# openxrlab/xrsfm

Hardware: AMD Instinct MI355X
Metric: BA iterations/sec x (cams+points) (higher is better)
Workload: dtype f64

## Files before the change

include/xrsfm_ba.h:

```cpp
#ifndef XRSFM_BA_H
#define XRSFM_BA_H

#include <stddef.h>
#include <stdint.h>

#ifdef __cplusplus
extern "C" {
#endif

#define XRSFM_BA_VERSION 1

#define XRSFM_BA_OK 0
#define XRSFM_BA_EINVAL (-1)
#define XRSFM_BA_ENODEV (-2)
#define XRSFM_BA_ENOMEM (-3)
#define XRSFM_BA_ECOMM (-4)
#define XRSFM_BA_ESTATE (-5)
#define XRSFM_BA_ETOOBIG (-6)
#define XRSFM_BA_EINTERNAL (-7)
#define XRSFM_BA_ESINGULAR (-8)

#define XRSFM_BA_SIMPLE_PINHOLE 0
#define XRSFM_BA_PINHOLE 1
#define XRSFM_BA_SIMPLE_RADIAL 2
// ... 121 lines not shown
    const int32_t *sc_a, *sc_b;
    const double *sc_s12;
} xrsfm_pg_problem;

typedef struct xrsfm_pg_options {
    int32_t max_iterations;
    double function_tolerance, parameter_tolerance, gradient_tolerance;
    double initial_radius;
    int32_t verbose;
    int32_t bounds_active_set;
} xrsfm_pg_options;

typedef struct xrsfm_pg_summary {
    double initial_cost, final_cost;
    int32_t iterations, n_successful, n_unsuccessful;
    int32_t termination;
} xrsfm_pg_summary;

void xrsfm_pg_default_options(xrsfm_pg_options *opt);
int xrsfm_pg_solve(const xrsfm_pg_options *opt, xrsfm_pg_problem *problem, xrsfm_pg_summary *summary);

typedef struct xrsfm_tag_problem {
    int32_t n_frames;
    const double *frame_q;
    const double *frame_t;
    int32_t n_tags;
    double tag_length;
    double *tag_corners;
    double *tag_q, *tag_t;
    double scale;
    double scale_lower;
    int32_t n_tag_obs;
    const int32_t *tag_obs_tag, *tag_obs_frame;
    const double *tag_obs_xy;
    int32_t n_points, n_obs;
    double *points;
    const int32_t *obs_frame, *obs_pt;
    const double *obs_xy;
} xrsfm_tag_problem;

void xrsfm_tag_default_options(xrsfm_pg_options *opt);
int xrsfm_tag_refine(const xrsfm_pg_options *opt, xrsfm_tag_problem *problem, int32_t stages, xrsfm_pg_summary *summaries);

int xrsfm_ba_filter_tracks(const xrsfm_ba_problem *problem, double max_reproj_error, double min_tri_angle_rad,
                           uint8_t *obs_delete, uint8_t *track_outlier, double *track_error, double *track_angle,
                           int32_t *num_filtered);

int xrsfm_ba_profile_entry(xrsfm_ba_context *ctx, int index, const char **name, double *total_ms, int *launches);


int xrsfm_ba_debug_linearize(xrsfm_ba_context *ctx, double huber_a, int use_scaling, double *r, double *Jc,
                             double *Jp, double *Hpp, double *gp, double *Hcc_diag, double *gc, double *cost);

int xrsfm_ba_debug_schur_product(xrsfm_ba_context *ctx, double radius, const double *x, double *y, double *b);

int xrsfm_ba_debug_pack(const xrsfm_ba_problem *problem, int32_t stats[8], int32_t *slot_obs);

int xrsfm_ba_debug_sgroup(const xrsfm_ba_problem *problem, int G, int32_t stats[3], int32_t *pos_tile, int32_t *pos_code,
                          int32_t *tile_stride, int32_t *tile_cams, int32_t *tile_cidx, int32_t *cam_ptr_s);
int xrsfm_ba_debug_pack_gram(const xrsfm_ba_problem *problem, int32_t stats[8], int32_t *tile_ncam, uint8_t *slot_cidx,
                             int32_t *slot_campos_g);

int xrsfm_ba_debug_gram_schedule(int n_cams, int32_t *n_inst, int32_t *n_inst_all, uint16_t *entries);

int xrsfm_ba_debug_chol_plan(const xrsfm_ba_problem *problem, int32_t stats[8], int32_t *cam_offset, int32_t *facts);

int xrsfm_ba_debug_device_pack_check(const xrsfm_ba_problem *problem, int32_t *field, int32_t *index);

int xrsfm_ba_debug_set_block_pattern(xrsfm_ba_context *ctx, int n_pairs, const int32_t *row_col);

int xrsfm_ba_debug_cholesky_solve(xrsfm_ba_context *ctx, double radius, double *y, double *S_dense);

int xrsfm_ba_debug_reduced_system(xrsfm_ba_context *ctx, double radius, int32_t facts[16], int32_t *n_blocks, int32_t *blk_rc,
                                  double *blk, double *diag, double *b, double *y);

int xrsfm_ba_debug_wide(xrsfm_ba_context *ctx, double huber_a, double radius, double *cost, double *r, double *Jc, double *Jp,
                        double *Hcc_diag, double *gc, double *y);

int xrsfm_ba_debug_backsub(xrsfm_ba_context *ctx, double *part_model, double *part_step2, double *cand_points,
                           double *point_step, double *cand_cam_q, double *cand_cam_t);

int xrsfm_ba_debug_stored_j(xrsfm_ba_context *ctx, int32_t *stored);

#ifdef __cplusplus
}
#endif
#endif
```

xrsfm_amd/capi.py:

```python
from __future__ import annotations

import ctypes as C
import os

import numpy as np

from . import _build

_c_double_p = C.POINTER(C.c_double)
_c_int32_p = C.POINTER(C.c_int32)
_c_uint8_p = C.POINTER(C.c_uint8)


class CProblem(C.Structure):
    _fields_ = [
        ("n_cams", C.c_int32), ("n_points", C.c_int32), ("n_obs", C.c_int32), ("n_intr", C.c_int32),
        ("cam_q", _c_double_p), ("cam_t", _c_double_p), ("cam_const", _c_uint8_p), ("cam_intr", _c_int32_p),
        ("intr_model", _c_int32_p), ("intr_params", _c_double_p),
        ("points", _c_double_p), ("point_const", _c_uint8_p),
        ("obs_cam", _c_int32_p), ("obs_pt", _c_int32_p), ("obs_uv", _c_double_p),
    ]


class CPgProblem(C.Structure):
    _fields_ = [("n_frames", C.c_int32), ("n_scales", C.c_int32), ("n_edges", C.c_int32), ("n_scale_costs", C.c_int32),
                ("rot_q", _c_double_p), ("pos", _c_double_p), ("scale", _c_double_p), ("pos_const", _c_uint8_p),
                ("scale_const", _c_uint8_p), ("scale_lower", _c_double_p), ("edge_a", _c_int32_p), ("edge_b", _c_int32_p),
                ("edge_sa", _c_int32_p), ("edge_sb", _c_int32_p), ("edge_q_mea", _c_double_p), ("edge_p_mea", _c_double_p),
                ("weight_o", C.c_double), ("sc_a", _c_int32_p), ("sc_b", _c_int32_p), ("sc_s12", _c_double_p)]


class CPgOptions(C.Structure):
    _fields_ = [("max_iterations", C.c_int32), ("function_tolerance", C.c_double), ("parameter_tolerance", C.c_double),
                ("gradient_tolerance", C.c_double), ("initial_radius", C.c_double), ("verbose", C.c_int32),
                ("bounds_active_set", C.c_int32)]


class CPgSummary(C.Structure):
    _fields_ = [("initial_cost", C.c_double), ("final_cost", C.c_double), ("iterations", C.c_int32), ("n_successful", C.c_int32),
                ("n_unsuccessful", C.c_int32), ("termination", C.c_int32)]


class CTagProblem(C.Structure):
    _fields_ = [("n_frames", C.c_int32), ("frame_q", _c_double_p), ("frame_t", _c_double_p), ("n_tags", C.c_int32),
                ("tag_length", C.c_double), ("tag_corners", _c_double_p), ("tag_q", _c_double_p), ("tag_t", _c_double_p),
                ("scale", C.c_double), ("scale_lower", C.c_double), ("n_tag_obs", C.c_int32), ("tag_obs_tag", _c_int32_p),
                ("tag_obs_frame", _c_int32_p), ("tag_obs_xy", _c_double_p), ("n_points", C.c_int32), ("n_obs", C.c_int32),
                ("points", _c_double_p), ("obs_frame", _c_int32_p), ("obs_pt", _c_int32_p), ("obs_xy", _c_double_p)]


ALLREDUCE_FN = C.CFUNCTYPE(C.c_int, C.c_void_p, C.POINTER(C.c_double), C.c_uint64, C.c_int)


class COptions(C.Structure):
    _fields_ = [
        ("max_iterations", C.c_int32), ("function_tolerance", C.c_double), ("parameter_tolerance", C.c_double),
        ("gradient_tolerance", C.c_double), ("initial_radius", C.c_double), ("huber_a", C.c_double),
        ("linear_solver", C.c_int32), ("pcg_tolerance", C.c_double), ("pcg_max_iterations", C.c_int32),
        ("profile", C.c_int32), ("verbose", C.c_int32),
    ]


class CSummary(C.Structure):
    _fields_ = [
        ("initial_cost", C.c_double), ("final_cost", C.c_double),
        ("num_residuals", C.c_int32), ("num_effective_params", C.c_int32),
        ("n_successful", C.c_int32), ("n_unsuccessful", C.c_int32),
        ("termination", C.c_int32), ("termination_reason", C.c_int32),
        ("pcg_iterations", C.c_int32), ("lm_steps_attempted", C.c_int32),
        ("total_time_s", C.c_double), ("dom_kernel_ms", C.c_double),
        ("dom_kernel_launches", C.c_int32), ("dom_kernel_id", C.c_int32),
        ("linear_solver_used", C.c_int32), ("reserved", C.c_int32),
    ]

    def as_dict(self):
        return {f: getattr(self, f) for f, _ in self._fields_}


EXPORTS = [
    "xrsfm_ba_default_options", "xrsfm_ba_version", "xrsfm_ba_create", "xrsfm_ba_comm_unique_id",
    "xrsfm_ba_comm_init", "xrsfm_ba_run", "xrsfm_ba_reset", "xrsfm_ba_download", "xrsfm_ba_destroy",
    "xrsfm_ba_solve", "xrsfm_ba_filter_tracks", "xrsfm_ba_profile_entry", "xrsfm_ba_debug_linearize", "xrsfm_ba_debug_schur_product",
    "xrsfm_ba_debug_cholesky_solve", "xrsfm_ba_debug_set_block_pattern", "xrsfm_ba_debug_pack", "xrsfm_ba_debug_chol_plan", "xrsfm_ba_refine_pose", "xrsfm_ba_refine_pose_options", "xrsfm_ba_debug_comm_hook", "xrsfm_pg_default_options", "xrsfm_pg_solve", "xrsfm_ba_debug_pack_gram", "xrsfm_ba_debug_gram_schedule",
    "xrsfm_tag_default_options", "xrsfm_tag_refine", "xrsfm_ba_refine_poses", "xrsfm_ba_quiesce", "xrsfm_ba_debug_backsub", "xrsfm_ba_device_memory", "xrsfm_ba_download_intrinsics", "xrsfm_ba_debug_wide",
    "xrsfm_ba_debug_device_pack_check", "xrsfm_ba_warmup", "xrsfm_ba_debug_stored_j", "xrsfm_ba_debug_sgroup",
    "xrsfm_ba_debug_reduced_system", "xrsfm_ba_covariance",
]

CHOL_FACTS = ("T", "levels", "ordering", "schedule", "macro_levels", "split_levels", "la_depth", "fill_rest", "rest_apart", "packed",
              "bwd", "height_mask", "cw", "blocks", "n", "tiles_nz")
SCHEDULES = ("level", "panel", "lookahead")
BWD_FORMS = ("fused", "per_level", "all", "chunk", "push")


def _facts(v) -> dict:
    f = dict(zip(CHOL_FACTS, (int(x) for x in v)))
    f["schedule"] = SCHEDULES[f["schedule"]]
    f["bwd"] = BWD_FORMS[f["bwd"]]
    f["rest_apart"] = bool(f["rest_apart"]); f["packed"] = bool(f["packed"])
    f["heights"] = sorted(m * f["cw"] for m in range(1, 31) if (f["height_mask"] >> m) & 1)
    return f

SOLVER_PCG, SOLVER_CHOLESKY, SOLVER_AUTO = 0, 1, 2

ERRORS = {-1: "EINVAL", -2: "ENODEV (no HIP device / HIP error; there is no CPU fallback)", -3: "ENOMEM",
          -4: "ECOMM", -5: "ESTATE", -6: "ETOOBIG", -7: "EINTERNAL (unexpected exception inside the library)",
          -8: "ESINGULAR (the undamped reduced camera matrix is not positive definite)"}
ESINGULAR = -8

_lib = None


def load(path: str | None = None):
    global _lib
    if _lib is not None:
        return _lib
    path = path or os.environ.get("XRSFM_BA_LIB") or _build.LIB
    if not os.path.exists(path):
        raise RuntimeError(f"{path} is missing: run __graft_entry__.build() (hipcc --offload-arch=gfx950); "
                           "the BA path has no fallback implementation")
    lib = C.CDLL(path, mode=C.RTLD_GLOBAL)
    vp = C.c_void_p
    lib.xrsfm_ba_default_options.argtypes = [C.POINTER(COptions)]; lib.xrsfm_ba_default_options.restype = None
    lib.xrsfm_ba_version.argtypes = [C.POINTER(C.c_int)]; lib.xrsfm_ba_version.restype = C.c_int
    lib.xrsfm_ba_create.argtypes = [C.POINTER(CProblem), C.c_int, C.POINTER(vp)]; lib.xrsfm_ba_create.restype = C.c_int
    lib.xrsfm_ba_comm_unique_id.argtypes = [C.c_char_p]; lib.xrsfm_ba_comm_unique_id.restype = C.c_int
    lib.xrsfm_ba_comm_init.argtypes = [vp, C.c_int, C.c_int, C.c_char_p]; lib.xrsfm_ba_comm_init.restype = C.c_int
    lib.xrsfm_ba_run.argtypes = [vp, C.POINTER(COptions), C.POINTER(CSummary)]; lib.xrsfm_ba_run.restype = C.c_int
    lib.xrsfm_ba_reset.argtypes = [vp]; lib.xrsfm_ba_reset.restype = C.c_int
    lib.xrsfm_ba_download.argtypes = [vp, _c_double_p, _c_double_p, _c_double_p]; lib.xrsfm_ba_download.restype = C.c_int
    lib.xrsfm_ba_destroy.argtypes = [vp]; lib.xrsfm_ba_destroy.restype = None
    lib.xrsfm_ba_solve.argtypes = [C.POINTER(COptions), C.POINTER(CProblem), C.POINTER(CSummary)]; lib.xrsfm_ba_solve.restype = C.c_int
    lib.xrsfm_ba_filter_tracks.argtypes = [C.POINTER(CProblem), C.c_double, C.c_double, _c_uint8_p, _c_uint8_p, _c_double_p,
                                            _c_double_p, _c_int32_p]
    lib.xrsfm_ba_filter_tracks.restype = C.c_int
    lib.xrsfm_ba_debug_linearize.argtypes = [vp, C.c_double, C.c_int] + [_c_double_p] * 8
    lib.xrsfm_ba_debug_linearize.restype = C.c_int
    lib.xrsfm_ba_debug_schur_product.argtypes = [vp, C.c_double, _c_double_p, _c_double_p, _c_double_p]
    lib.xrsfm_ba_debug_schur_product.restype = C.c_int
    lib.xrsfm_ba_debug_cholesky_solve.argtypes = [vp, C.c_double, _c_double_p, _c_double_p]
    lib.xrsfm_ba_debug_cholesky_solve.restype = C.c_int
    if hasattr(lib, "xrsfm_ba_debug_stored_j"):
        lib.xrsfm_ba_debug_stored_j.argtypes = [vp, C.POINTER(C.c_int32)]
        lib.xrsfm_ba_debug_stored_j.restype = C.c_int
    if hasattr(lib, "xrsfm_ba_debug_backsub"):
        lib.xrsfm_ba_debug_backsub.argtypes = [vp] + [_c_double_p] * 6
        lib.xrsfm_ba_debug_backsub.restype = C.c_int
    lib.xrsfm_ba_debug_set_block_pattern.argtypes = [vp, C.c_int, _c_int32_p]
    lib.xrsfm_ba_debug_set_block_pattern.restype = C.c_int
    lib.xrsfm_pg_default_options.argtypes = [C.POINTER(CPgOptions)]
    lib.xrsfm_pg_default_options.restype = None
    lib.xrsfm_ba_refine_poses.argtypes = [C.POINTER(COptions), C.c_int32, _c_int32_p, _c_double_p, _c_int32_p, _c_double_p, _c_double_p,
                                          _c_uint8_p, _c_double_p, _c_double_p, C.POINTER(CSummary)]
    lib.xrsfm_ba_refine_poses.restype = C.c_int
    lib.xrsfm_pg_solve.argtypes = [C.POINTER(CPgOptions), C.POINTER(CPgProblem), C.POINTER(CPgSummary)]
    lib.xrsfm_pg_solve.restype = C.c_int
    lib.xrsfm_tag_default_options.argtypes = [C.POINTER(CPgOptions)]
    lib.xrsfm_tag_default_options.restype = None
    lib.xrsfm_tag_refine.argtypes = [C.POINTER(CPgOptions), C.POINTER(CTagProblem), C.c_int32, C.POINTER(CPgSummary)]
    lib.xrsfm_tag_refine.restype = C.c_int
    lib.xrsfm_ba_debug_comm_hook.argtypes = [C.c_void_p, C.c_int, C.c_int, ALLREDUCE_FN, C.c_void_p]
    lib.xrsfm_ba_debug_comm_hook.restype = C.c_int
    lib.xrsfm_ba_refine_pose_options.argtypes = [C.POINTER(COptions)]
    lib.xrsfm_ba_refine_pose_options.restype = None
    lib.xrsfm_ba_refine_pose.argtypes = [C.POINTER(COptions), C.c_int32, _c_double_p, C.c_int32, _c_double_p, _c_double_p, _c_uint8_p,
                                         _c_double_p, _c_double_p, C.POINTER(CSummary)]
    lib.xrsfm_ba_refine_pose.restype = C.c_int
    lib.xrsfm_ba_debug_pack_gram.argtypes = [C.POINTER(CProblem), _c_int32_p, _c_int32_p, _c_uint8_p, _c_int32_p]
    lib.xrsfm_ba_debug_pack_gram.restype = C.c_int
    lib.xrsfm_ba_debug_sgroup.argtypes = [C.POINTER(CProblem), C.c_int] + [_c_int32_p] * 7
    lib.xrsfm_ba_debug_sgroup.restype = C.c_int
    lib.xrsfm_ba_debug_chol_plan.argtypes = [C.POINTER(CProblem), _c_int32_p, _c_int32_p, _c_int32_p]
    lib.xrsfm_ba_debug_chol_plan.restype = C.c_int
    lib.xrsfm_ba_debug_reduced_system.argtypes = [vp, C.c_double, _c_int32_p, C.POINTER(C.c_int32), _c_int32_p] + [_c_double_p] * 4
    lib.xrsfm_ba_debug_reduced_system.restype = C.c_int
    lib.xrsfm_ba_debug_pack.argtypes = [C.POINTER(CProblem), _c_int32_p, _c_int32_p]
    lib.xrsfm_ba_debug_pack.restype = C.c_int
    lib.xrsfm_ba_profile_entry.argtypes = [vp, C.c_int, C.POINTER(C.c_char_p), _c_double_p, C.POINTER(C.c_int)]
    lib.xrsfm_ba_profile_entry.restype = C.c_int
    lib.xrsfm_ba_covariance.argtypes = [vp, C.c_double, C.c_int32, _c_int32_p, _c_double_p]
    lib.xrsfm_ba_covariance.restype = C.c_int
    _lib = lib
    return lib


def check(code: int, what: str):
    if code != 0:
        raise RuntimeError(f"{what} failed: {code} {ERRORS.get(code, '')}")


def _dp(a):
    return a.ctypes.data_as(_c_double_p) if a is not None else None


def device_count() -> int:
    n = C.c_int(0)
    load().xrsfm_ba_version(C.byref(n))
    return n.value


def quiesce() -> int:
    n = C.c_uint64(0)
    lib = load()
    lib.xrsfm_ba_quiesce.argtypes = [C.POINTER(C.c_uint64)]
    lib.xrsfm_ba_quiesce.restype = C.c_int
    check(lib.xrsfm_ba_quiesce(C.byref(n)), "xrsfm_ba_quiesce")
    return int(n.value)


def default_options(**kw) -> COptions:
    o = COptions()
    load().xrsfm_ba_default_options(C.byref(o))
    for k, v in kw.items():
        if not hasattr(o, k):
            raise AttributeError(k)
        setattr(o, k, v)
    return o


class ProblemArrays:
    FIELDS = ("cam_q", "cam_t", "cam_const", "cam_intr", "intr_model", "intr_params",
              "points", "point_const", "obs_cam", "obs_pt", "obs_uv")

    def __init__(self, **arr):
        f64 = lambda a, s: np.ascontiguousarray(np.asarray(a, np.float64).reshape(s))
        self.cam_q = f64(arr["cam_q"], (-1, 4)); self.cam_t = f64(arr["cam_t"], (-1, 3))
        n_c = self.cam_q.shape[0]
        cc = arr.get("cam_const")
        self.cam_const = np.ascontiguousarray(np.zeros(n_c, np.uint8) if cc is None else np.asarray(cc, np.uint8))
        self.cam_intr = np.ascontiguousarray(np.asarray(arr["cam_intr"], np.int32))
        self.intr_model = np.ascontiguousarray(np.asarray(arr["intr_model"], np.int32))
        self.intr_params = f64(arr["intr_params"], (-1, 8))
        self.points = f64(arr["points"], (-1, 3))
        pc = arr.get("point_const")
        self.point_const = np.ascontiguousarray(np.zeros(self.points.shape[0], np.uint8) if pc is None else np.asarray(pc, np.uint8))
        self.obs_cam = np.ascontiguousarray(np.asarray(arr["obs_cam"], np.int32))
        self.obs_pt = np.ascontiguousarray(np.asarray(arr["obs_pt"], np.int32))
        self.obs_uv = f64(arr["obs_uv"], (-1, 2))
        if not (self.cam_t.shape[0] == n_c and self.cam_intr.shape[0] == n_c and self.cam_const.shape[0] == n_c):
            raise ValueError("cam_q / cam_t / cam_intr / cam_const disagree on the number of cameras")
        if not (self.obs_pt.shape[0] == self.obs_cam.shape[0] == self.obs_uv.shape[0]):
            raise ValueError("obs_cam / obs_pt / obs_uv disagree on the number of observations")
        if self.point_const.shape[0] != self.points.shape[0] or self.intr_model.shape[0] != self.intr_params.shape[0]:
            raise ValueError("point_const / points or intr_model / intr_params disagree in length")

    @property
    def n_cams(self): return self.cam_q.shape[0]
    @property
    def n_points(self): return self.points.shape[0]
    @property
    def n_obs(self): return self.obs_cam.shape[0]

    def as_dict(self):
        return {k: getattr(self, k) for k in self.FIELDS}

    def c_struct(self) -> CProblem:
        i32 = lambda a: a.ctypes.data_as(_c_int32_p)
        u8 = lambda a: a.ctypes.data_as(_c_uint8_p)
        return CProblem(self.n_cams, self.n_points, self.n_obs, self.intr_model.shape[0],
                        _dp(self.cam_q), _dp(self.cam_t), u8(self.cam_const), i32(self.cam_intr),
                        i32(self.intr_model), _dp(self.intr_params), _dp(self.points), u8(self.point_const),
                        i32(self.obs_cam), i32(self.obs_pt), _dp(self.obs_uv))


class Context:

    def __init__(self, problem: ProblemArrays, device: int = 0):
        self.lib = load()
        self.problem = problem
        self._h = C.c_void_p()
        cs = problem.c_struct()
        check(self.lib.xrsfm_ba_create(C.byref(cs), device, C.byref(self._h)), "xrsfm_ba_create")

    def close(self):
        if self._h:
            self.lib.xrsfm_ba_destroy(self._h)
            self._h = C.c_void_p()

    def __del__(self):
        try:
            self.close()
        except Exception:
            pass

    def comm_init(self, n_ranks: int, rank: int, unique_id: bytes):
        check(self.lib.xrsfm_ba_comm_init(self._h, n_ranks, rank, unique_id), "xrsfm_ba_comm_init")

    def comm_hook(self, n_ranks: int, rank: int, allreduce):
        def _cb(user, buf, n, op):
            try:
                allreduce(np.ctypeslib.as_array(buf, shape=(int(n),)), int(op))
                return 0
            except Exception:
                return 1
        self._hook = ALLREDUCE_FN(_cb)
        check(self.lib.xrsfm_ba_debug_comm_hook(self._h, n_ranks, rank, self._hook, None), "xrsfm_ba_debug_comm_hook")

    def run(self, options: COptions | None = None) -> CSummary:
        options = options or default_options()
        s = CSummary()
        check(self.lib.xrsfm_ba_run(self._h, C.byref(options), C.byref(s)), "xrsfm_ba_run")
        return s

    def reset(self):
        check(self.lib.xrsfm_ba_reset(self._h), "xrsfm_ba_reset")

    def download(self, out=None):
        p = self.problem
        if out is None:
            q = np.empty_like(p.cam_q); t = np.empty_like(p.cam_t); P = p.points.copy()
        else:
            q, t, P = out
            if not (q.shape == p.cam_q.shape and t.shape == p.cam_t.shape and P.shape == p.points.shape):
                raise ValueError("download(out=...): shapes must equal the problem's cam_q / cam_t / points")
            if not all(a.dtype == np.float64 and a.flags.c_contiguous and a.flags.writeable for a in (q, t, P)):
                raise ValueError("download(out=...): arrays must be writable C-contiguous float64")
            if P is not p.points:
                P[...] = p.points
        check(self.lib.xrsfm_ba_download(self._h, _dp(q), _dp(t), _dp(P)), "xrsfm_ba_download")
        return q, t, P

    def covariance(self, cams, huber_a: float = 5.99) -> np.ndarray:
        sel = np.ascontiguousarray(cams, np.int32).reshape(-1)
        cov = np.zeros((sel.shape[0], 6, 6))
        check(self.lib.xrsfm_ba_covariance(self._h, huber_a, sel.shape[0], sel.ctypes.data_as(_c_int32_p), _dp(cov)), "xrsfm_ba_covariance")
        return cov

    def debug_linearize(self, huber_a: float = 5.99, use_scaling: bool = False):
        p = self.problem
        out = dict(r=np.zeros((p.n_obs, 2)), Jc=np.zeros((p.n_obs, 2, 6)), Jp=np.zeros((p.n_obs, 2, 3)),
                   Hpp=np.zeros((p.n_points, 6)), gp=np.zeros((p.n_points, 3)),
                   Hcc_diag=np.zeros((p.n_cams, 6)), gc=np.zeros((p.n_cams, 6)))
        cost = C.c_double(0)
        check(self.lib.xrsfm_ba_debug_linearize(self._h, huber_a, int(use_scaling), _dp(out["r"]), _dp(out["Jc"]),
                                                _dp(out["Jp"]), _dp(out["Hpp"]), _dp(out["gp"]), _dp(out["Hcc_diag"]),
                                                _dp(out["gc"]), C.cast(C.byref(cost), _c_double_p)), "debug_linearize")
        out["cost"] = cost.value
        return out

    def debug_schur_product(self, radius: float, x: np.ndarray):
        x = np.ascontiguousarray(x, np.float64)
        y = np.zeros_like(x); b = np.zeros_like(x)
        check(self.lib.xrsfm_ba_debug_schur_product(self._h, radius, _dp(x), _dp(y), _dp(b)), "debug_schur_product")
        return y, b


    def debug_stored_j(self) -> bool:
        v = C.c_int32(0)
        check(self.lib.xrsfm_ba_debug_stored_j(self._h, C.byref(v)), "debug_stored_j")
        return bool(v.value)

    def debug_cholesky_solve(self, radius: float, want_S: bool = False):
        n = 6 * self.problem.n_cams
        y = np.zeros((self.problem.n_cams, 6))
        S = np.zeros((n, n)) if want_S else None
        check(self.lib.xrsfm_ba_debug_cholesky_solve(self._h, radius, _dp(y), _dp(S)), "debug_cholesky_solve")
        return y, S

    def debug_reduced_system(self, radius: float, want_y: bool = True) -> dict:
        import scipy.sparse as sp
        lib = self.lib
        facts = np.zeros(16, np.int32)
        nb = C.c_int32(0)
        check(lib.xrsfm_ba_debug_reduced_system(self._h, radius, facts.ctypes.data_as(_c_int32_p), C.byref(nb), None, None, None, None, None),
              "xrsfm_ba_debug_reduced_system")
        f = _facts(facts)
        nc, cw, m = self.problem.n_cams, f["cw"], nb.value
        rc = np.zeros((max(m, 1), 2), np.int32); blk = np.zeros((max(m, 1), cw, cw)); diag = np.zeros((nc, cw, cw)); b = np.zeros((nc, cw))
        y = np.zeros((nc, cw)) if want_y else None
        check(lib.xrsfm_ba_debug_reduced_system(self._h, radius, facts.ctypes.data_as(_c_int32_p), C.byref(nb), rc.ctypes.data_as(_c_int32_p),
                                                _dp(blk), _dp(diag), _dp(b), _dp(y)), "xrsfm_ba_debug_reduced_system")
        rc, blk = rc[:m], blk[:m]
        ar = np.arange(cw)
        def coo(rows, cols, vals):
            shape = (len(rows), cw, cw)
            r = np.broadcast_to(cw * rows[:, None, None] + ar[None, :, None], shape)
            c = np.broadcast_to(cw * cols[:, None, None] + ar[None, None, :], shape)
            return r.ravel(), c.ravel(), vals.ravel()
        cams = np.arange(nc)
        parts = [coo(cams, cams, diag), coo(rc[:, 0], rc[:, 1], blk), coo(rc[:, 1], rc[:, 0], blk.transpose(0, 2, 1))]
        r, c, v = (np.concatenate(x) for x in zip(*parts))
        S = sp.csr_matrix((v, (r, c)), shape=(nc * cw, nc * cw))
        return dict(S=S, b=b, y=y, facts=f, blk_rc=rc)

    def download_intrinsics(self) -> np.ndarray:
        out = np.array(self.problem.intr_params, copy=True)
        self.lib.xrsfm_ba_download_intrinsics.argtypes = [C.c_void_p, _c_double_p]
        self.lib.xrsfm_ba_download_intrinsics.restype = C.c_int
        check(self.lib.xrsfm_ba_download_intrinsics(self._h, _dp(out)), "xrsfm_ba_download_intrinsics")
        return out

    def debug_wide(self, huber_a: float = 5.99, radius: float | None = None) -> dict:
        p = self.problem
        out = dict(r=np.zeros((p.n_obs, 2)), Jc=np.zeros((p.n_obs, 2, 9)), Jp=np.zeros((p.n_obs, 2, 3)), Hcc_diag=np.zeros((p.n_cams, 9)),
                   gc=np.zeros((p.n_cams, 9)))
        y = np.zeros((p.n_cams, 9)) if radius is not None else None
        cost = C.c_double(0)
        self.lib.xrsfm_ba_debug_wide.argtypes = [C.c_void_p, C.c_double, C.c_double, C.POINTER(C.c_double)] + [_c_double_p] * 6
        self.lib.xrsfm_ba_debug_wide.restype = C.c_int
        check(self.lib.xrsfm_ba_debug_wide(self._h, huber_a, float(radius or 1.0), C.byref(cost), _dp(out["r"]), _dp(out["Jc"]), _dp(out["Jp"]),
                                          _dp(out["Hcc_diag"]), _dp(out["gc"]), _dp(y)), "xrsfm_ba_debug_wide")
        out["cost"] = cost.value
        if y is not None:
            out["y"] = y
        return out

    def debug_backsub(self) -> dict:
        st = debug_pack(self.problem)
        ni, npk, nc = st["items"], st["active_points"], self.problem.n_cams
        out = dict(part_model=np.zeros(ni), part_step2=np.zeros(ni), cand_points=np.zeros((npk, 3)), point_step=np.zeros((npk, 3)),
                   cand_cam_q=np.zeros((nc, 4)), cand_cam_t=np.zeros((nc, 3)))
        check(self.lib.xrsfm_ba_debug_backsub(self._h, *[_dp(out[k]) for k in ("part_model", "part_step2", "cand_points", "point_step",
                                                                                  "cand_cam_q", "cand_cam_t")]), "debug_backsub")
        return out

    def debug_set_block_pattern(self, row_col: np.ndarray):
        rc = np.ascontiguousarray(row_col, np.int32).reshape(-1, 2)
        check(self.lib.xrsfm_ba_debug_set_block_pattern(self._h, rc.shape[0], rc.ctypes.data_as(_c_int32_p)), "debug_set_block_pattern")

    def profile(self) -> dict:
        out = {}
        i = 0
        while True:
            name = C.c_char_p(); ms = C.c_double(0); n = C.c_int(0)
            if self.lib.xrsfm_ba_profile_entry(self._h, i, C.byref(name), C.cast(C.byref(ms), _c_double_p), C.byref(n)) != 0:
                break
            out[name.value.decode()] = (ms.value, n.value)
            i += 1
        return out


def comm_unique_id() -> bytes:
    buf = C.create_string_buffer(128)
# ... 219 lines not shown
```

xrsfm_amd/csrc/ba_chol.h:

```cpp
#pragma once
#include "ba_kernels.h"
#include "ba_pack.h"

namespace xba {

constexpr int kNB = 64;
constexpr int kLdT = 66;
constexpr int kCamsPerTileDev = 10;

struct CholDev {
    int n, n_pad, T;
    double* S;
    const int* tmap; size_t ld; size_t tstride;
    double* Linv;
    double* y;
    double* rhs;
    double* x;
    const int* cam_off;
    const int* tile_rows;
    int cw, cpt;
};

__device__ __forceinline__ double* tile_ptr(const CholDev& c, int i, int k) {
    return c.tmap ? c.S + (size_t)c.tmap[i * c.T + k] * c.tstride : c.S + (size_t)(i * kNB) * c.ld + k * kNB;
// ... 204 lines not shown
    lds_ptr pb[NB];
    double acc[NB];
    lds_ptr Vb = (lds_ptr)Vst + 8 * kk;
#pragma unroll
    for (int u = 0; u < NB; ++u) {
        const int rg = e[u] & 255, cg = e[u] >> 8;
        pa[u] = Vb + 8 * (min(4 * rg + i4, R - 1) * Cp);
        pb[u] = Vb + 8 * (min(4 * cg + i4, R - 1) * Cp);
        acc[u] = 0.0;
    }
    int k0 = 0;
    for (; k0 + 16 <= C4; k0 += 16) {
#pragma unroll
        for (int j = 0; j < 4; ++j)
#pragma unroll
            for (int u = 0; u < NB; ++u)
                acc[u] = __builtin_amdgcn_mfma_f64_4x4x4f64(*(lds_dptr)(pa[u] + 32 * j), *(lds_dptr)(pb[u] + 32 * j), acc[u], 0, 0, 0);
#pragma unroll
        for (int u = 0; u < NB; ++u) { pa[u] += 128; pb[u] += 128; }
    }
    for (; k0 < C4; k0 += 4) {
#pragma unroll
        for (int u = 0; u < NB; ++u) {
            acc[u] = __builtin_amdgcn_mfma_f64_4x4x4f64(*(lds_dptr)pa[u], *(lds_dptr)pb[u], acc[u], 0, 0, 0);
            pa[u] += 32; pb[u] += 32;
        }
    }
    if (sg.len > 1 && !sgroup_finish(sg, acc, scat, lane)) return;
    int dst[NB];
    unsigned off[NB];
#pragma unroll
    for (int u = 0; u < NB; ++u) {
        const unsigned row = 4u * (unsigned)(e[u] & 255) + (unsigned)kk, col = 4u * (unsigned)(e[u] >> 8) + (unsigned)i4;
        const unsigned rb = gram_cam_of_row<CW>(row), ra = gram_cam_of_row<CW>(col);
        dst[u] = dtab[ra * kGramTabLd + rb];
        off[u] = CW * (row - CW * rb) + (col - CW * ra);
    }
#pragma unroll
    for (int u = 0; u < NB; ++u)
        if (dst[u] >= 0) scat2[(unsigned long long)(unsigned)dst[u] * (unsigned)(CW * CW) + off[u]] = acc[u];
}

template <int CW = 6>
__device__ __forceinline__ void gram_tile4(double* __restrict__ Vst, int R, int Cp, int C, const int* __restrict__ dtab,
                                           double* __restrict__ scat2, int lane, const double (&V)[3 * CW], bool valid, int t, int cidx,
                                           int T, bool dense, const unsigned short* __restrict__ sched, int n_inst, SGroup sg,
                                           double* __restrict__ scat) {
    const unsigned short* ent = sched + ((lane >> 2) & 3);
    const int C4 = (3 * T + 3) & ~3;
    if (dense) {
        const int padc = C4 - 3 * T;
        for (int e = lane; e < R * padc; e += kWave) {
            const int row = e / padc, cc = 3 * T + (e - row * padc);
            Vst[row * Cp + cc] = 0.0;
        }
    } else {
        for (int e = lane; e < (R * Cp) / 2; e += kWave) reinterpret_cast<double2*>(Vst)[e] = make_double2(0.0, 0.0);
        if (((R * Cp) & 1) && lane == kWave - 1) Vst[R * Cp - 1] = 0.0;
    }
    if (valid) {
#pragma unroll
        for (int i = 0; i < CW; ++i)
#pragma unroll
            for (int m = 0; m < 3; ++m) Vst[(CW * cidx + i) * Cp + 3 * t + m] = V[3 * i + m];
    }
    __builtin_amdgcn_s_waitcnt(0xc07f);
    __builtin_amdgcn_wave_barrier();
    XBA_STAMP(0, 6);
    switch (n_inst) {
        case 6: gram4_batch<CW, 6>(Vst, R, Cp, C4, ent, dtab, scat2, lane, sg, scat); break;
        case 5: gram4_batch<CW, 5>(Vst, R, Cp, C4, ent, dtab, scat2, lane, sg, scat); break;
        case 4: gram4_batch<CW, 4>(Vst, R, Cp, C4, ent, dtab, scat2, lane, sg, scat); break;
        case 3: gram4_batch<CW, 3>(Vst, R, Cp, C4, ent, dtab, scat2, lane, sg, scat); break;
        case 2: gram4_batch<CW, 2>(Vst, R, Cp, C4, ent, dtab, scat2, lane, sg, scat); break;
        default: gram4_batch<CW, 1>(Vst, R, Cp, C4, ent, dtab, scat2, lane, sg, scat); break;
    }
    XBA_STAMP(0, 7);
}

template <bool GRAM, bool PREP, int NIK>
__global__ __launch_bounds__((GRAM && NIK == 0) ? kWave * kSGroupMax : kWave) __attribute__((amdgpu_waves_per_eu((GRAM && NIK < 4) ? 4 : (GRAM ? 3 : 2), (GRAM && NIK < 4) ? 4 : 3)))
void k_schur_pairs(Dev d, const int* __restrict__ item_list, const int* __restrict__ slot_pair_ptr, const int* __restrict__ pair_dst,
                   int n_obs_pairs, double* __restrict__ scat2, double radius, double* __restrict__ pair_v = nullptr, int gram4 = 1,
                   const int* __restrict__ sgrp = nullptr, int n_list = 0, int wld = 0) {
    extern __shared__ __attribute__((aligned(16))) double smem_all[];
    constexpr bool MERGED = GRAM && NIK == 0;
    const int lane = MERGED ? (int)__builtin_amdgcn_mbcnt_hi(~0u, __builtin_amdgcn_mbcnt_lo(~0u, 0u)) : (int)threadIdx.x;
    const int wave = MERGED ? __builtin_amdgcn_readfirstlane((int)(threadIdx.x >> 6)) : 0;
    const int pos = MERGED ? (int)blockIdx.x * (int)(blockDim.x >> 6) + wave : (int)blockIdx.x;
    if (MERGED && pos >= n_list) return;
    double* const smem = smem_all + (size_t)wave * wld;
    XBA_STAMP(0, 0);
    SGroup sg{0, 1, smem, wld, 0.0, 0.0, -1};
    if (MERGED && sgrp) {
        const int code = __builtin_amdgcn_readfirstlane(sgrp[pos]);
        sg.idx = code & 15; sg.len = code >> 4;
    }
    const int entry = item_list[MERGED ? n_list - 1 - pos : pos];
    Item it;
    if (GRAM) { it.first_tile = entry; it.n_tiles = 1; }
    else it = d.items[entry];
    if (GRAM || it.n_tiles == 1) {
        int dt0 = -1, dt1 = -1;
        int g4_se = 0, g4_n = 0;
        if (GRAM) {
            const int C0 = d.tile_ncam[it.first_tile];
            const int* src = pair_dst + n_obs_pairs + d.tile_gt_off[it.first_tile];
            const int a0 = lane / kGramTabLd, b0 = lane - kGramTabLd * a0;
            const int a1 = (lane + kWave) / kGramTabLd, b1 = lane + kWave - kGramTabLd * a1;
            if (b0 > a0 && b0 < C0) dt0 = src[a0 * C0 + b0];
            if (b1 > a1 && b1 < C0 && a1 < kGramTabLd) dt1 = src[a1 * C0 + b1];
            if (NIK <= 2 && gram4) g4_se = gram4_sched_load<6>(C0, lane, g4_n);
        }
        const SlotCtx s = load_slot(d, it.first_tile, lane);
        const int cp = d.slot_campos_s[s.slot];
        const int cidx_raw = GRAM ? (int)d.slot_cidx[s.slot] : 0;
        const int L = d.tile_stride[it.first_tile];
        int g_pos = kWave - 1, g_pk0 = 0, g_pk1 = 0, g_pk2 = 0;
        if (GRAM && L == 0) {
            const int C0 = d.tile_ncam[it.first_tile];
            const int* trun = d.tile_run + (size_t)it.first_tile * kTileRunLd;
            const int c0 = lane / 14, c1 = (lane + 64) / 14, c2 = (lane + 128) / 14;
            g_pos = (int)d.slot_gpos[s.slot];
            if (c0 < C0) g_pk0 = trun[c0];
            if (c1 < C0) g_pk1 = trun[c1];
            if (c2 < C0) g_pk2 = trun[c2];
        }
        double V[18];
        int npair = 0, pbase = 0;
        {
            double o28[28];
            XBA_STAMP(0, 1);
            if (s.valid) {
                double hcv[6], gv[3];
                {
                    const double* hc = (PREP ? d.Hpp : d.Hc) + 6 * (size_t)s.pt;
                    const double* g = d.gp + 3 * (size_t)s.pt;
#pragma unroll
                    for (int k = 0; k < 6; ++k) hcv[k] = hc[k];
                    gv[0] = g[0]; gv[1] = g[1]; gv[2] = g[2];
                }
                double F[12], E[6], r0, r1;
                load_FE_rc(d, s.slot, s.cam, s.pt, F, E, r0, r1);
                if (PREP) { double hf[6]; point_factor(hcv, radius, hf);
#pragma unroll
                    for (int k = 0; k < 6; ++k) hcv[k] = hf[k]; }
                XBA_STAMP(0, 2);
                pairs_V<PREP>(F, E, hcv, V);
                XBA_STAMP(0, 3);
                pairs_diag<PREP>(F, V, hcv, gv, o28);
            } else if (PREP) { dead_values(V); dead_values(o28); }
            else {
#pragma unroll
                for (int k = 0; k < 18; ++k) V[k] = XBA_DEAD;
#pragma unroll
                for (int k = 0; k < 28; ++k) o28[k] = XBA_DEAD;
            }
            XBA_STAMP(0, 4);
            const int Cg = GRAM ? d.tile_ncam[it.first_tile] : 0;
            if (L > 0) {
                const int T = __popcll(__ballot(s.valid)) / L;
                double* red = smem;
#pragma unroll
                for (int h = 0; h < 2; ++h) {
#pragma unroll
                    for (int k = 0; k < 14; ++k) red[lane * kRedLd + k] = o28[14 * h + k];
                    __builtin_amdgcn_s_waitcnt(0xc07f);
                    __builtin_amdgcn_wave_barrier();
                    if ((L == 4 && T == 16) || (L == 2 && T == 32) || (L == 3 && T == 21)) {
// ... 1394 lines not shown
```

xrsfm_amd/csrc/ba_kernels.h:

```cpp
#pragma once
#include "ba_math.h"

namespace xba {

constexpr int kWave = 64;
constexpr int kBlock = 256;
constexpr int kWavesPerBlock = kBlock / kWave;

struct Item { int first_tile; int n_tiles; };

struct PcgStatus {
    double rz;
    double rr;
    double bb;
    double pq;
    int it;
    int done;
    unsigned arrived;
};

enum Scal {
    S_COST = 0, S_XNORM2_PTS, S_MODEL, S_STEP2_PTS, S_COST_CAND, S_STEP2_CAMS, S_XNORM2_CAMS,
    S_GRADMAX_PTS, S_GRADMAX_CAMS,
    S_BWD_ERR,
    S_COUNT = 16
};

struct __attribute__((aligned(16))) CamLin {
    double M[9];
    double sq[3];
    double st[3];
    double pad;
};
static_assert(sizeof(CamLin) == 128, "CamLin must be 128 bytes");

struct Dev {
    int n_cams, n_pts, n_tiles, n_slots, n_items;
    const int* slot_cam; const int* slot_pt; const int* slot_campos;
    const double* slot_u; const double* slot_v;
    const Item* items;
    const int* tile_stride;
    const int* tile_maxlen;
    const int* tile_ncam;
    const int* tile_gt_off;
    const unsigned char* slot_cidx;
    const int* slot_campos_g;
    const unsigned char* slot_gpos;
    const int* tile_run;
    const int* cam_ptr_g;
    const int* slot_campos_s; const int* cam_ptr_s;
    CamRec* cam; CamRec* cam_cand; const int* cam_model; const unsigned char* cam_const; const int* cam_ptr;
    double* cam_act;
    double* P; double* P_cand; const unsigned char* pt_const;
    double* scale_c; double* scale_p;
    double* rt; double* Jp;
    double huber_a;
    CamLin* camrec;
    double* Hpp; double* gp; double* Hinv;
    double* Hc;
    double* camlin;
    double* Dc2;
    double* camS;
    double* Minv;
    double* b;
    double* px; double* pr; double* pz; double* pp; double* pq;
    double* yp;
    double* scat;
    double* part;
    double* campart;
    double* ptpart;
    double* pcgpart;
    double* pcgW;
    double* pcgSW;
    double* pcgE;
    double* scal;
    PcgStatus* st;
};

#ifdef XBA_TIMELINE
__device__ unsigned long long g_stamps[3][64][16];
#define XBA_STAMP(kern, i) do { if ((threadIdx.x & 63) == 0 && (blockIdx.x % 97) == 0 && blockIdx.x / 97 < 64 && (threadIdx.x >> 6) == 0) g_stamps[kern][blockIdx.x / 97][i] = __builtin_readcyclecounter(); } while (0)
#define XBA_STAMP_W1(kern, i) do { if ((threadIdx.x & 63) == 0 && (blockIdx.x % 97) == 0 && blockIdx.x / 97 < 64 && (threadIdx.x >> 6) == 1) g_stamps[kern][blockIdx.x / 97][i] = __builtin_readcyclecounter(); } while (0)
#else
#define XBA_STAMP(kern, i) do {} while (0)
#define XBA_STAMP_W1(kern, i) do {} while (0)
#endif

#ifdef XBA_POISON
#define XBA_DEAD (__builtin_nan(""))
#define XBA_DEAD1 (__builtin_nan(""))
#define XBA_DEAD_VALUE(x) ((x) = __builtin_nan(""))
#else
#define XBA_DEAD 0.0
#define XBA_DEAD1 1.0
#define XBA_DEAD_VALUE(x) asm volatile("" : "=v"(x))
#endif
template <int N> __device__ __forceinline__ void dead_values(double (&v)[N]) {
#pragma unroll
    for (int k = 0; k < N; ++k) XBA_DEAD_VALUE(v[k]);
}
#ifndef XBA_BACKSUB_WAVES
#define XBA_BACKSUB_WAVES 0
#endif

__device__ __forceinline__ double wave_sum(double v) {
#pragma unroll
    for (int off = 32; off > 0; off >>= 1) v += __shfl_down(v, off, kWave);
    return v;
}
// ... 390 lines not shown
    xn2 = wave_sum(xn2);
#pragma unroll
    for (int off = 32; off > 0; off >>= 1) gm = fmax(gm, __shfl_xor(gm, off, kWave));
    if (lane == 0) { d.part[item] = cost; d.part[d.n_items + item] = xn2; d.part[2 * (size_t)d.n_items + item] = gm; }
}

__global__ __launch_bounds__(kBlock) __attribute__((amdgpu_waves_per_eu(4, 4))) void k_linearize(Dev d, double huber_a) {
    const int lane = threadIdx.x & (kWave - 1);
    const int item = __builtin_amdgcn_readfirstlane(blockIdx.x * kWavesPerBlock + (threadIdx.x >> 6));
    if (item >= d.n_items) return;
    const Item it = d.items[item];
    if (it.n_tiles > 1) linearize_item<true>(d, it, item, lane, huber_a);
    else linearize_item<false>(d, it, item, lane, huber_a);
}

__global__ __launch_bounds__(kBlock) void k_cost(Dev d, double huber_a) {
    const int lane = threadIdx.x & (kWave - 1);
    const int item = __builtin_amdgcn_readfirstlane(blockIdx.x * kWavesPerBlock + (threadIdx.x >> 6));
    if (item >= d.n_items) return;
    const Item it = d.items[item];
    double cost = 0.0;
    for (int tl = 0; tl < it.n_tiles; ++tl) {
        const int slot = (it.first_tile + tl) * kWave + lane;
        const int cam = d.slot_cam[slot];
        if (cam >= 0) {
            const CamRec& c = d.cam_cand[cam];
            double q[4] = {c.q[0], c.q[1], c.q[2], c.q[3]};
            double t[3] = {c.t[0], c.t[1], c.t[2]};
            const double* P = d.P_cand + 3 * (size_t)d.slot_pt[slot];
            const double Pw[3] = {P[0], P[1], P[2]};
            double M[9];
            quat_to_mat(q, M);
            Proj pr;
            project<false>(M, t, c.intr, d.cam_model[cam], Pw, d.slot_u[slot], d.slot_v[slot], pr);
            double rho1;
            cost += huber(pr.r0 * pr.r0 + pr.r1 * pr.r1, huber_a, rho1);
        }
    }
    cost = wave_sum(cost);
    if (lane == 0) d.part[item] = cost;
}

template <int K, bool WT = false>
__device__ __forceinline__ void segsum_body(const double* __restrict__ scat, const int* __restrict__ ptr, double* __restrict__ out, int c,
                                            double* lds_out = nullptr) {
    constexpr int G = kBlock / K;
    __shared__ double lds[G * K];
    const int t = threadIdx.x;
    const int beg = ptr[c], end = ptr[c + 1];
    if (t < G * K) {
        const int g = t / K;
        double acc = 0.0;
        const double* base = scat + (size_t)beg * K + t;
        const int n = end - beg;
        int o = g;
        for (; o + 3 * G < n; o += 4 * G) {
            const double v0 = base[0], v1 = base[(size_t)G * K], v2 = base[(size_t)2 * G * K], v3 = base[(size_t)3 * G * K];
            acc += v0; acc += v1; acc += v2; acc += v3;
            base += (size_t)4 * G * K;
        }
        for (; o < n; o += G) { acc += *base; base += (size_t)G * K; }
        lds[t] = acc;
    }
    __syncthreads();
    if (t < K) {
        double s = 0.0;
#pragma unroll 4
        for (int g = 0; g < G; ++g) s += lds[g * K + t];
        if (WT) __hip_atomic_store(out + (size_t)c * K + t, s, __ATOMIC_RELAXED, __HIP_MEMORY_SCOPE_AGENT);
        else out[(size_t)c * K + t] = s;
        if (lds_out) lds_out[t] = s;
    }
}

template <int K>
__global__ __launch_bounds__(kBlock) void k_cam_segsum(const double* __restrict__ scat, const int* __restrict__ cam_ptr,
                                                       double* __restrict__ out, const PcgStatus* st) {
    if (st && st->done) return;
    segsum_body<K>(scat, cam_ptr, out, blockIdx.x);
}

__global__ __launch_bounds__(kBlock) void k_chol_segsum(const double* __restrict__ scat, const int* __restrict__ cam_ptr,
                                                        double* __restrict__ camS, int n_cams, const double* __restrict__ scat2,
                                                        const int* __restrict__ blk_ptr, double* __restrict__ Sblk) {
    if ((int)blockIdx.x < n_cams) segsum_body<28>(scat, cam_ptr, camS, blockIdx.x);
    else segsum_body<36>(scat2, blk_ptr, Sblk, blockIdx.x - n_cams);
}

__global__ __launch_bounds__(kWave) void k_pair_sources(Dev d, const int* __restrict__ item_list, const int* __restrict__ slot_pair_ptr,
                                                        const int* __restrict__ pair_dst, int2* __restrict__ ent_src) {
    const Item it = d.items[item_list[blockIdx.x]];
    const int s_begin = it.first_tile * kWave, s_end = s_begin + it.n_tiles * kWave;
    for (int sa = s_begin + (int)threadIdx.x; sa < s_end; sa += kWave) {
        if (d.slot_cam[sa] < 0) continue;
        const int pbase = slot_pair_ptr[sa], npair = slot_pair_ptr[sa + 1] - pbase;
        for (int dd = 1; dd <= npair; ++dd) ent_src[pair_dst[pbase + dd - 1]] = make_int2(sa, sa + dd);
    }
}
__global__ __launch_bounds__(256) void k_gram_compact_count(const int* __restrict__ cell_dst, int n_cells, int* __restrict__ block_cnt) {
    const int i = blockIdx.x * 256 + threadIdx.x;
    const bool on = i < n_cells && cell_dst[i] >= 0;
    const int c = __syncthreads_count(on);
    if (threadIdx.x == 0) block_cnt[blockIdx.x] = c;
}
__global__ void k_gram_compact_scan(int* __restrict__ block_cnt, int n_blocks) {
    if (blockIdx.x != 0 || threadIdx.x != 0) return;
    int run = 0;
    for (int b = 0; b < n_blocks; ++b) { const int v = block_cnt[b]; block_cnt[b] = run; run += v; }
}
__global__ __launch_bounds__(256) void k_gram_compact(int* __restrict__ cell_dst, int n_cells, int2* __restrict__ ent_src, const int* __restrict__ block_off) {
    __shared__ int wave_cnt[4];
    const int i = blockIdx.x * 256 + threadIdx.x, lane = threadIdx.x & 63, wave = threadIdx.x >> 6;
    const int e = i < n_cells ? cell_dst[i] : -1;
    const unsigned long long m = __ballot(e >= 0);
    if (lane == 0) wave_cnt[wave] = __popcll(m);
    __syncthreads();
    if (e < 0) return;
    int rec = block_off[blockIdx.x] + __popcll(m & ((1ull << lane) - 1ull));
    for (int w = 0; w < wave; ++w) rec += wave_cnt[w];
    ent_src[e] = make_int2(-1, rec);
    cell_dst[i] = rec;
}
constexpr int kPairVAhead = 8;
__global__ __launch_bounds__(kBlock) void k_chol_segsum_v(const double* __restrict__ scat, const int* __restrict__ cam_ptr,
                                                          double* __restrict__ camS, int n_cams, const double* __restrict__ scat2,
                                                          const int* __restrict__ blk_ptr, double* __restrict__ Sblk, int n_blocks,
                                                          const int2* __restrict__ ent_src, const double* __restrict__ pair_v) {
    if ((int)blockIdx.x < n_cams) { segsum_body<28>(scat, cam_ptr, camS, blockIdx.x); return; }
    constexpr int K = 36, NW = kBlock / kWave;
    __shared__ double ops[NW][kPairVAhead][K];
    const int t = threadIdx.x, lane = t & (kWave - 1);
    const int wave = __builtin_amdgcn_readfirstlane(t >> 6);
    const int b = ((int)blockIdx.x - n_cams) * NW + wave;
    if (b >= n_blocks) return;
    const int beg = blk_ptr[b], end = blk_ptr[b + 1];
    const int k = lane < K ? lane : 0, rb3 = 3 * (k / 6), ca3 = 3 * (k % 6);
    double acc = 0.0;
    for (int e0 = beg; e0 < end; e0 += kPairVAhead) {
        const int2 mine = (lane < kPairVAhead && e0 + lane < end) ? ent_src[e0 + lane] : make_int2(-1, -1);
        int sx[kPairVAhead], sy[kPairVAhead];
        double v[kPairVAhead];
#pragma unroll
        for (int u = 0; u < kPairVAhead; ++u) {
            sx[u] = __builtin_amdgcn_readlane(mine.x, u); sy[u] = __builtin_amdgcn_readlane(mine.y, u);
            v[u] = 0.0;
            if (e0 + u < end && lane < K)
                v[u] = sx[u] < 0 ? scat2[36 * (size_t)sy[u] + lane] : pair_v[18 * (size_t)(lane < 18 ? sx[u] : sy[u]) + (lane < 18 ? lane : lane - 18)];
        }
#pragma unroll
        for (int u = 0; u < kPairVAhead; ++u) {
            if (e0 + u >= end) break;
            if (sx[u] < 0) { acc += v[u]; continue; }
            double* row = ops[wave][u];
            if (lane < K) row[lane] = v[u];
            __builtin_amdgcn_s_waitcnt(0xc07f);
            __builtin_amdgcn_wave_barrier();
            const double* Va = row + ca3;
            const double* Vb = row + 18 + rb3;
            acc += Vb[0] * Va[0] + Vb[1] * Va[1] + Vb[2] * Va[2];
        }
    }
    if (lane < K) Sblk[(size_t)b * K + lane] = acc;
}

__global__ void k_debug_materialize(Dev d, double* __restrict__ Fs, double* __restrict__ Es) {
    const int slot = blockIdx.x * blockDim.x + threadIdx.x;
    if (slot >= d.n_slots || d.slot_cam[slot] < 0) return;
    double F[12], E[6], r0, r1;
    load_FE_rc(d, slot, d.slot_cam[slot], d.slot_pt[slot], F, E, r0, r1);
    const size_t ns = (size_t)d.n_slots;
    for (int k = 0; k < 12; ++k) Fs[k * ns + slot] = F[k];
    for (int k = 0; k < 6; ++k) Es[k * ns + slot] = E[k];
}

__global__ void k_materialize_rj(Dev d, double* __restrict__ rt, double* __restrict__ Jp) {
    const int slot = blockIdx.x * blockDim.x + threadIdx.x;
    if (slot >= d.n_slots || d.slot_cam[slot] < 0) return;
    const int cam = d.slot_cam[slot];
    const CamLin& c = d.camrec[cam];
    double M[9];
    for (int k = 0; k < 9; ++k) M[k] = c.M[k];
    const double* P = d.P + 3 * (size_t)d.slot_pt[slot];
    const double Pw[3] = {P[0], P[1], P[2]};
    double r0, r1, j[6];
    obs_rj(d, slot, cam, M, Pw, r0, r1, j);
    const size_t ns = (size_t)d.n_slots;
    if (rt) { rt[slot] = r0; rt[ns + slot] = r1; }
    if (Jp) for (int k = 0; k < 6; ++k) Jp[k * ns + slot] = j[k];
}

__global__ void k_scale_from_norms(Dev d) {
    const int i = blockIdx.x * blockDim.x + threadIdx.x;
    if (i < d.n_cams * 6) {
        const int c = i / 6, k = i % 6;
        d.scale_c[i] = 1.0 / (1.0 + sqrt(d.camlin[12 * (size_t)c + k]));
    }
    if (i < d.n_pts * 3) {
        const int p = i / 3, k = i % 3;
        const int di = (k == 0) ? 0 : (k == 1 ? 3 : 5);
        d.scale_p[i] = 1.0 / (1.0 + sqrt(d.Hpp[6 * (size_t)p + di]));
    }
}

__global__ void k_fill(double* p, double v, size_t n) {
    const size_t i = (size_t)blockIdx.x * blockDim.x + threadIdx.x;
    if (i < n) p[i] = v;
}

__global__ void k_point_prep(Dev d, double radius, double dmin, double dmax, int n_pt_blocks) {
    if ((int)blockIdx.x >= n_pt_blocks) {
// ... 747 lines not shown
    if (threadIdx.x == 0) {
        double r = 0.0;
        for (int i = 0; i < kPcgThreads / kWave; ++i) r = fmax(r, lds[i]);
        *out = r;
        if (rank_max) {
            double m2 = 0.0;
            for (int i = 0; i < n_ranks; ++i) m2 = fmax(m2, rank_max[i]);
            *out_pts = m2;
        }
    }
}

struct ReduceJobs { const double* in[8]; int n[8]; double* out[8]; int op[8]; };

__global__ __launch_bounds__(kPcgThreads) void k_reduce_sum(const double* __restrict__ in, int n, double* out) {
    __shared__ double lds[kPcgThreads / kWave];
    double s = 0.0;
    for (int i = threadIdx.x; i < n; i += kPcgThreads) s += in[i];
    s = block_sum<kPcgThreads>(s, lds);
    if (threadIdx.x == 0) *out = s;
}

__global__ __launch_bounds__(kPcgThreads) void k_reduce_multi(ReduceJobs jobs) {
    __shared__ double lds[kPcgThreads / kWave];
    const double* in = jobs.in[blockIdx.x];
    const int n = jobs.n[blockIdx.x];
    if (jobs.op[blockIdx.x] == 0) {
        double s = 0.0;
        int i = threadIdx.x;
        for (; i + 7 * kPcgThreads < n; i += 8 * kPcgThreads) {
            double v[8];
#pragma unroll
            for (int u = 0; u < 8; ++u) v[u] = in[i + u * kPcgThreads];
            s += ((v[0] + v[1]) + (v[2] + v[3])) + ((v[4] + v[5]) + (v[6] + v[7]));
        }
        for (; i < n; i += kPcgThreads) s += in[i];
        s = block_sum<kPcgThreads>(s, lds);
        if (threadIdx.x == 0) *jobs.out[blockIdx.x] = s;
    } else {
        double m = 0.0;
        int i = threadIdx.x;
        for (; i + 7 * kPcgThreads < n; i += 8 * kPcgThreads) {
            double v[8];
#pragma unroll
            for (int u = 0; u < 8; ++u) v[u] = in[i + u * kPcgThreads];
#pragma unroll
            for (int u = 0; u < 8; ++u) m = fmax(m, v[u]);
        }
        for (; i < n; i += kPcgThreads) m = fmax(m, in[i]);
#pragma unroll
        for (int off = 32; off > 0; off >>= 1) m = fmax(m, __shfl_down(m, off, kWave));
        if ((threadIdx.x & 63) == 0) lds[threadIdx.x >> 6] = m;
        __syncthreads();
        if (threadIdx.x == 0) {
            double r = 0.0;
            for (int i2 = 0; i2 < kPcgThreads / kWave; ++i2) r = fmax(r, lds[i2]);
            *jobs.out[blockIdx.x] = r;
        }
    }
}

__global__ __launch_bounds__(kPcgThreads) void k_reduce_max(const double* __restrict__ in, int n, double* out) {
    __shared__ double lds[kPcgThreads / kWave];
    double m = 0.0;
    for (int i = threadIdx.x; i < n; i += kPcgThreads) m = fmax(m, in[i]);
#pragma unroll
    for (int off = 32; off > 0; off >>= 1) m = fmax(m, __shfl_down(m, off, kWave));
    if ((threadIdx.x & 63) == 0) lds[threadIdx.x >> 6] = m;
    __syncthreads();
    if (threadIdx.x == 0) {
        double r = 0.0;
        for (int i = 0; i < kPcgThreads / kWave; ++i) r = fmax(r, lds[i]);
        *out = r;
    }
}

constexpr int kTailGrid = 1024;
struct TailArgs {
    ReduceJobs jobs; int njobs;
    double* part2;
    unsigned* ticket;
    int gradmax;
    double* host; unsigned long long seq;
};

constexpr int kTailJobs = 8;

__global__ __launch_bounds__(kBlock) void k_lin_tail(Dev d, TailArgs a) {
    __shared__ double sums[12];
    __shared__ double sc[S_COUNT];
    __shared__ bool last;
    const int t = threadIdx.x, lane = t & 63, wave = t >> 6, G = gridDim.x, b = blockIdx.x;
    double gm = 0.0;
    for (int c = b; c < d.n_cams; c += G) {
        __syncthreads();
        segsum_body<12, true>(d.scat, d.cam_ptr_g, d.camlin, c, sums);
        __syncthreads();
        if (t == 0 && a.gradmax) gm = fmax(gm, cam_gradmax_one(d, c, sums + 6));
    }
    if (t == 0 && a.gradmax) __hip_atomic_store(a.part2 + (size_t)(kTailJobs - 1) * G + b, gm, __ATOMIC_RELAXED, __HIP_MEMORY_SCOPE_AGENT);
    for (int j = wave; j < a.njobs; j += kBlock / kWave) {
        const double* in = a.jobs.in[j];
        const int n = a.jobs.n[j], op = a.jobs.op[j];
        const int len = (n + G - 1) / G, lo = min(n, b * len), hi = min(n, lo + len);
        double v = 0.0;
        for (int i = lo + lane; i < hi; i += kWave) v = (op == 0) ? v + in[i] : fmax(v, in[i]);
        if (op == 0) v = wave_sum(v);
        else {
#pragma unroll
            for (int off = 32; off > 0; off >>= 1) v = fmax(v, __shfl_down(v, off, kWave));
        }
        if (lane == 0) __hip_atomic_store(a.part2 + (size_t)j * G + b, v, __ATOMIC_RELAXED, __HIP_MEMORY_SCOPE_AGENT);
    }
    asm volatile("s_waitcnt vmcnt(0)" ::: "memory");
    __syncthreads();
    if (t == 0) {
        const int sh = b & 7, nsh = min(G, 8), n_in_shard = (G - sh + 7) >> 3;
        bool l = false;
        if (__hip_atomic_fetch_add(a.ticket + 32 * sh, 1u, __ATOMIC_RELAXED, __HIP_MEMORY_SCOPE_AGENT) + 1u == (unsigned)n_in_shard)
            l = (__hip_atomic_fetch_add(a.ticket + 32 * 8, 1u, __ATOMIC_RELAXED, __HIP_MEMORY_SCOPE_AGENT) + 1u == (unsigned)nsh);
        last = l;
    }
    __syncthreads();
    if (!last) return;
    __builtin_amdgcn_fence(__ATOMIC_ACQUIRE, "agent");
    if (t < S_COUNT) sc[t] = __hip_atomic_load(d.scal + t, __ATOMIC_RELAXED, __HIP_MEMORY_SCOPE_AGENT);
    __syncthreads();
    {
        const int j = t >> 5, l32 = t & 31;
        const bool isgm = (j == kTailJobs - 1);
        const bool on = isgm ? (a.gradmax != 0) : (j < a.njobs);
        const int op = isgm ? 1 : (on ? a.jobs.op[j] : 0);
        const double* in = a.part2 + (size_t)j * G;
        double v = 0.0;
        if (on)
            for (int i0 = l32; i0 < G; i0 += 32 * 8) {
                double x[8];
#pragma unroll
                for (int u = 0; u < 8; ++u) { const int i = i0 + 32 * u; x[u] = (i < G) ? in[i] : 0.0; }
#pragma unroll
                for (int u = 0; u < 8; ++u)
                    if (i0 + 32 * u < G) v = (op == 0) ? v + x[u] : fmax(v, x[u]);
            }
#pragma unroll
        for (int off = 16; off > 0; off >>= 1) {
            const double ov = __shfl_down(v, off, 32);
            v = (op == 0) ? v + ov : fmax(v, ov);
        }
        if (on && l32 == 0) {
            double* out = isgm ? d.scal + S_GRADMAX_CAMS : a.jobs.out[j];
            *out = v;
            const long long idx = out - d.scal;
            if (idx >= 0 && idx < S_COUNT) sc[idx] = v;
        }
    }
    __syncthreads();
    if (t < 9) __hip_atomic_store(a.ticket + 32 * t, 0u, __ATOMIC_RELAXED, __HIP_MEMORY_SCOPE_AGENT);
    if (a.host) {
        if (t < S_COUNT) a.host[t] = sc[t];
        __threadfence_system();
        __syncthreads();
        if (t == 0)
            __hip_atomic_store(reinterpret_cast<unsigned long long*>(a.host + S_COUNT), a.seq, __ATOMIC_RELEASE, __HIP_MEMORY_SCOPE_SYSTEM);
    }
}

}
```

xrsfm_amd/csrc/ba_trust_region.h:

```cpp
#pragma once

#include <cmath>

#ifdef __HIPCC__
#define XTR_HD __host__ __device__
#else
#define XTR_HD
#endif

namespace xtr {

constexpr double kMaxRadius = 1e16;
constexpr double kMinRadius = 1e-32;
constexpr double kMinRelDecrease = 1e-3;
constexpr int kMaxInvalidSteps = 5;

struct TrustRegion {
    double radius;
    double decrease = 2.0;
    int invalid = 0;

    XTR_HD int invalid_step() {
        if (++invalid >= kMaxInvalidSteps) return 6;
        radius /= decrease; decrease *= 2.0;
        return 0;
    }
    XTR_HD static int tolerance_exit(double step_norm, double xnorm, double ptol, double cost_change, double cost, double ftol) {
        if (step_norm <= ptol * (xnorm + ptol)) return 2;
        if (std::fabs(cost_change) <= ftol * cost) return 3;
        return 0;
    }
    XTR_HD static bool successful(double rho) { return rho > kMinRelDecrease; }
    XTR_HD void grow(double rho) {
        radius = std::fmin(kMaxRadius, radius / std::fmax(1.0 / 3.0, 1.0 - std::pow(2.0 * rho - 1.0, 3)));
        decrease = 2.0;
    }
    XTR_HD int shrink() {
        radius /= decrease; decrease *= 2.0;
        return radius < kMinRadius ? 4 : 0;
    }
};

}
```

xrsfm_amd/csrc/xrsfm_ba.hip:

```cpp
#include <dlfcn.h>
#include <hip/hip_runtime.h>

#include <algorithm>
#include <chrono>
#include <condition_variable>
#include <deque>
#include <cmath>
#include <cstdio>
#include <cstdlib>
#include <cstring>
#include <map>
#include <mutex>
#include <thread>
#include <type_traits>
#include <vector>

#include "../../include/xrsfm_ba.h"
#include "ba_chol.h"
#include "ba_cov.h"
#include "ba_filter.h"
#include "ba_kernels.h"
#include "ba_pack.h"
#include "ba_plan.h"
#include "ba_refine.h"
// ... 66 lines not shown
    int *slot_pair_ptr = nullptr, *pair_dst = nullptr, *blk_ptr = nullptr, *blk_rc = nullptr;
    double *scat2 = nullptr, *Sblk = nullptr;
    bool bwd_push = false;
    bool bwd_chunk = false; int4* bc_chunks = nullptr; std::vector<int> bc_off; double* bc_part = nullptr; unsigned* bc_ctr = nullptr;
    int gram4 = 1;
    bool pair_from_v = false; int2* ent_src = nullptr; double* pair_v = nullptr;
    int* tiles_nz = nullptr;
    size_t pairs_shm = 0, pairs_shm_big = 0;
    int* pairs_items = nullptr; int n_pairs_small = 0, n_pairs_big = 0, n_pairs_other = 0;
    int gram_n[8] = {0}; size_t gram_shm[8] = {0};
    bool gram_merge = true;
    int sgroup = 1; int* sgrp = nullptr;
    hipStream_t aux = nullptr; hipEvent_t ev_fork = nullptr, ev_join = nullptr;
    int* cols_flat = nullptr;
    std::vector<int> cols_off;
    int* bw2_ent = nullptr; std::vector<int> bw2_off, bw2_link;
    bool use_levels = false, panel_ll = false;
    bool lookahead = false;
    int n_levels = 0;
    int *lv_k = nullptr, *lv_tgt = nullptr, *lv_cptr = nullptr, *lv_cj = nullptr;
    int *lv_bptr = nullptr, *lv_bi = nullptr;
    std::vector<int> lv_k_off, lv_tgt_off;
    int* bw_order = nullptr; unsigned char* bw_final = nullptr; unsigned long long* bw_gx = nullptr; unsigned* bw_ctr = nullptr;
    bool bw_debug_timeout = false;
    int bw_n = 0; unsigned bw_launches = 0; bool bwd_all = false;
    int *sp_tgt = nullptr, *sp_q = nullptr, *sp_rt = nullptr, *sp_rp = nullptr;
    int* sp_slot = nullptr;
    int la_depth = 0; std::vector<int> sp_e_cnt; std::vector<hipEvent_t> la_ev_factor, la_ev_early;
    std::vector<int> sp_chunk_off, sp_rt_off, mp_off;
    int *mp_chunk = nullptr, *mp_wg = nullptr;
    double* sp_work = nullptr; int sp_max_chunks = 0;
    int *fz_tile = nullptr, *fz_dptr = nullptr, *fz_dj = nullptr, *tile_cam = nullptr;
    int *md_tgt = nullptr, *md_q = nullptr, *md_cj = nullptr, *fz_late = nullptr;
    std::vector<int> md_off; int md_max = 0; double* md_work = nullptr;
    int *fz_q = nullptr, *fill_rest = nullptr; int n_fill_rest = 0;
    bool rest_apart = false;
    int32_t facts[16] = {0};
    bool S_filled = false;
    std::vector<int> fz_off;
    int *tf_ptr = nullptr, *tf_ent = nullptr;
    std::vector<int> cam_off_host;
    std::vector<int> tile_map_host; size_t S_doubles = 0;
    std::vector<int> lv_k_host, lv_bptr_host, lv_bi_host;
    int ordering = 0;
};

struct xrsfm_ba_context {
    int device = 0;
    hipStream_t stream = nullptr;
    Packed pk;
    Dev d{};
    std::vector<void*> allocs;
    std::vector<size_t> alloc_class;
    CamRec* cam0 = nullptr; double* P0 = nullptr;
    int n_points_caller = 0;
    double* h_scal = nullptr;
    double* h_scal_dev = nullptr;
    unsigned long long seq = 0;
    PcgStatus* h_st = nullptr;
    void* comm = nullptr; int n_ranks = 1, rank = 0;
    xrsfm_ba_allreduce_fn hook = nullptr; void* hook_user = nullptr; std::vector<double> hook_buf;
    bool multi() const { return comm != nullptr || hook != nullptr; }
    bool profiling = false;
    std::vector<hipEvent_t> ev_pool; size_t ev_used = 0;
    struct Rec { int kid; size_t e0; int tag; };
    std::vector<Rec> recs;
    double prof_ms[K_COUNT] = {0}; int prof_n[K_COUNT] = {0};
    bool dev_packed = false; int host_pack_level = 2;
    int* dpk_slot_obs = nullptr; unsigned char* dpk_gt_cell = nullptr;
    bool linearized = false;
    unsigned long long debug_stall_ticks = 0;
    bool poisoned = false;
    bool fused = true;
    bool wide = false;
    DevW w{};
    std::vector<int> cam_intr_host;
    bool pcg_coarse = true; double* pcg_w = nullptr;
    bool prep_fused = true;
    double step_radius = 0.0;
    bool step_prep = false;
    bool step_valid = false;
    bool gradmax_done = false, published = false;
    double* part2 = nullptr; unsigned* ticket = nullptr;
    struct LinBuf { double* rt = nullptr; double* Jp = nullptr; CamLin* camrec = nullptr; double* Hpp = nullptr; double* gp = nullptr; double* camlin = nullptr; } alt;
    double* jbuf[4] = {nullptr, nullptr, nullptr, nullptr};
    std::vector<unsigned long long> pattern_keys;
    bool have_pattern = false;
    CholHost chol;
};

namespace {

struct DevCache {
    std::mutex mu;
    std::map<std::pair<int, size_t>, std::vector<void*>> free_blocks;
    size_t cached_bytes = 0;
    static size_t size_class(size_t bytes) {
        size_t c = 256;
        while (c < bytes) c += (c < (1u << 20)) ? c : c / 4;
        return c;
    }
    void* get(int dev, size_t bytes, size_t* cls) {
        *cls = size_class(bytes);
        {
            std::lock_guard<std::mutex> g(mu);
            auto it = free_blocks.find({dev, *cls});
            if (it != free_blocks.end() && !it->second.empty()) { void* p = it->second.back(); it->second.pop_back(); cached_bytes -= *cls; return p; }
        }
        void* p = nullptr;
        if (hipMalloc(&p, *cls) != hipSuccess) {
            release_all();
            if (hipMalloc(&p, *cls) != hipSuccess) return nullptr;
        }
        return p;
    }
    void put(int dev, void* p, size_t cls) {
        std::lock_guard<std::mutex> g(mu);
        if (cached_bytes + cls > (size_t)16 << 30) { (void)hipFree(p); return; }
        free_blocks[{dev, cls}].push_back(p); cached_bytes += cls;
    }
    void release_all() {
        std::lock_guard<std::mutex> g(mu);
        for (auto& kv : free_blocks) for (void* p : kv.second) (void)hipFree(p);
        free_blocks.clear(); cached_bytes = 0;
    }
};
DevCache g_cache;

struct HostBundle { hipStream_t stream; double* h_scal; PcgStatus* h_st; hipStream_t aux = nullptr; hipEvent_t ev_fork = nullptr, ev_join = nullptr; };
static void bundle_release(const HostBundle& b) {
    (void)hipHostFree(b.h_scal); (void)hipHostFree(b.h_st); (void)hipStreamDestroy(b.stream);
    if (b.aux) { (void)hipStreamDestroy(b.aux); (void)hipEventDestroy(b.ev_fork); (void)hipEventDestroy(b.ev_join); }
}
struct BundleCache {
    std::mutex mu;
    std::map<int, std::vector<HostBundle>> free_bundles;
    bool get(int dev, HostBundle* b) {
        {
            std::lock_guard<std::mutex> g(mu);
            auto& v = free_bundles[dev];
            if (!v.empty()) { *b = v.back(); v.pop_back(); return true; }
        }
        *b = HostBundle{nullptr, nullptr, nullptr};
        if (hipStreamCreate(&b->stream) != hipSuccess) return false;
        if (hipHostMalloc((void**)&b->h_scal, sizeof(double) * (S_COUNT + 2), hipHostMallocMapped | hipHostMallocCoherent) != hipSuccess ||
            hipHostMalloc((void**)&b->h_st, sizeof(PcgStatus)) != hipSuccess) {
            if (b->h_scal) (void)hipHostFree(b->h_scal);
            (void)hipStreamDestroy(b->stream);
            return false;
        }
        return true;
    }
    void put(int dev, const HostBundle& b) {
        std::lock_guard<std::mutex> g(mu);
        auto& v = free_bundles[dev];
        if (v.size() >= 8) { bundle_release(b); return; }
        v.push_back(b);
    }
};
BundleCache g_bundles;

struct PinnedPool {
    std::mutex mu;
    std::vector<std::pair<void*, size_t>> free_blocks;
    void* get(size_t bytes, size_t* cap) {
        {
// ... 197 lines not shown
    }
    const unsigned long long* flag = reinterpret_cast<const unsigned long long*>(c->h_scal + S_COUNT);
    static const double watchdog_env = [] { const char* e = std::getenv("XRSFM_BA_WATCHDOG_S"); return e ? std::atof(e) : -1.0; }();
    const double watchdog_s = watchdog_env >= 0.0 ? watchdog_env : (c->multi() ? 300.0 : 0.0);
    std::chrono::steady_clock::time_point t_wait{};
    bool waiting = false;
    for (unsigned spins = 0; __atomic_load_n(flag, __ATOMIC_ACQUIRE) != want; ++spins) {
        if ((spins & 0xfffff) == 0xfffff) {
            const hipError_t q = hipStreamQuery(c->stream);
            if (q == hipSuccess) { if (__atomic_load_n(flag, __ATOMIC_ACQUIRE) == want) break; return XRSFM_BA_ENODEV; }
            if (q != hipErrorNotReady) return XRSFM_BA_ENODEV;
            const auto now = std::chrono::steady_clock::now();
            if (!waiting) { waiting = true; t_wait = now; }
            else if (watchdog_s > 0.0 && std::chrono::duration<double>(now - t_wait).count() > watchdog_s) {
                fprintf(stderr, "[xrsfm_ba] rank %d of %d: the device has made no progress for %.0f s%s\n", c->rank, c->n_ranks, watchdog_s,
                        c->multi() ? " — an all-reduce that never completed? every rank must make the same calls in the same order (XRSFM_BA_WATCHDOG_S)" : "");
                c->poisoned = true;
                return c->multi() ? XRSFM_BA_ECOMM : XRSFM_BA_ENODEV;
            }
        }
        __builtin_ia32_pause();
    }
    return bwd_err_check(c);
}

constexpr int kJfreeMinSlots = 1 << 20;
int jfree_setting() {
    const char* e = std::getenv("XRSFM_BA_JFREE");
    return e ? (e[0] == '0' ? 0 : 1) : -1;
}
bool jfree_enabled() { return jfree_setting() != 0; }
int use_stored_j(xrsfm_ba_context* c, bool on, bool materialize = false) {
    Dev& d = c->d;
    if (!on) { d.rt = d.Jp = c->alt.rt = c->alt.Jp = nullptr; return 0; }
    if (d.Jp) return 0;
    const size_t ns = (size_t)d.n_slots;
    for (int i = 0; i < 4; ++i) {
        if (c->jbuf[i]) continue;
        if (int e = dev_alloc(c, &c->jbuf[i], ns * (i & 1 ? 6 : 2))) { c->jbuf[i] = nullptr; return e; }
    }
    d.rt = c->jbuf[0]; d.Jp = c->jbuf[1]; c->alt.rt = c->jbuf[2]; c->alt.Jp = c->jbuf[3];
    if (materialize && ns) {
        hipLaunchKernelGGL(k_materialize_rj, dim3(cdiv((long long)ns, kBlock)), dim3(kBlock), 0, c->stream, d, d.rt, d.Jp);
        if (hipGetLastError() != hipSuccess) return XRSFM_BA_ENODEV;
    }
    return 0;
}

bool jfree_for_run(const xrsfm_ba_context* c, int solver) {
    const int set = jfree_setting();
    return solver == XRSFM_BA_SOLVER_CHOLESKY && !c->wide && c->chol.n_pairs_other == 0 && (set == 1 || (set < 0 && c->d.n_slots >= kJfreeMinSlots));
}

enum { LIN_SKIP_CAMLIN = 1, LIN_FINAL = 2 };
int linearize(xrsfm_ba_context* c, double huber_a, const Dev& d, bool with_step, int flags = 0) {
    const Dev& own = c->d;
    c->gradmax_done = false; c->published = false;
    c->step_valid = false;
    c->d.huber_a = huber_a;
    if (d.n_cams > 0 && !(flags & LIN_SKIP_CAMLIN)) LAUNCH(c, K_SMALL, k_cam_lin, dim3(cdiv(d.n_cams, kBlock)), dim3(kBlock), 0, d);
    if (d.n_items > 0) LAUNCH(c, K_LINEARIZE, k_linearize, dim3(cdiv(d.n_items, kWavesPerBlock)), dim3(kBlock), kWavesPerBlock * kWave * 13 * sizeof(double), d, huber_a);
    if (!c->fused && d.n_cams > 0) LAUNCH(c, K_CAM_SEGSUM, k_cam_segsum<12>, dim3(d.n_cams), dim3(kBlock), 0, d.scat, d.cam_ptr_g, d.camlin, (const PcgStatus*)nullptr);
    {
        double* tail = d.camlin + (size_t)d.n_cams * 12;
        const bool multi = c->multi();
        ReduceJobs j{};
        int nj = 0;
        auto job = [&](const double* in, int n, double* out, int op) { j.in[nj] = in; j.n[nj] = n; j.out[nj] = out; j.op[nj] = op; ++nj; };
        job(d.part, d.n_items, multi ? tail : d.scal + S_COST, 0);
        job(d.part + d.n_items, d.n_items, multi ? tail + 1 : d.scal + S_XNORM2_PTS, 0);
        job(d.part + 2 * (size_t)d.n_items, d.n_items, multi ? tail + 4 + c->rank : d.scal + S_GRADMAX_PTS, 1);
        if (with_step) {
            job(own.part + 2 * (size_t)own.n_items, own.n_items, multi ? tail + 2 : d.scal + S_MODEL, 0);
            job(own.part + 3 * (size_t)own.n_items, own.n_items, multi ? tail + 3 : d.scal + S_STEP2_PTS, 0);
            job(own.campart, own.n_cams, d.scal + S_STEP2_CAMS, 0);
            job(own.campart + own.n_cams, own.n_cams, d.scal + S_XNORM2_CAMS, 0);
        }
        if (multi) HIPCHK(hipMemsetAsync(tail + 2, 0, sizeof(double) * (2 + (size_t)c->n_ranks), c->stream));
        if (c->fused) {
            TailArgs a{};
            a.jobs = j; a.njobs = nj; a.part2 = c->part2; a.ticket = c->ticket;
            const bool final_here = (flags & LIN_FINAL) && !multi;
            a.gradmax = final_here ? 1 : 0;
            if (final_here && !c->profiling && c->h_scal_dev) { a.host = c->h_scal_dev; a.seq = ++c->seq; c->published = true; }
            LAUNCH(c, K_SMALL, k_lin_tail, dim3(std::min(kTailGrid, std::max(d.n_cams, 1))), dim3(kBlock), 0, d, a);
            if (final_here) c->gradmax_done = true;
        } else {
            LAUNCH(c, K_SMALL, k_reduce_multi, dim3(nj), dim3(kPcgThreads), 0, j);
        }
        if (multi) {
            int e = allreduce(c, d.camlin, (size_t)d.n_cams * 12 + 4 + (size_t)c->n_ranks, kNcclSum);
            if (e) return e;
            HIPCHK(hipMemcpyAsync(d.scal + S_COST, tail, 4 * sizeof(double), hipMemcpyDeviceToDevice, c->stream));
        }
    }
    return 0;
}

int linearize_wide(xrsfm_ba_context* c, double huber_a) {
    if (int e = use_stored_j(c, true)) return e;
    Dev& d = c->d;
    c->gradmax_done = false; c->published = false;
    if (d.n_items > 0) LAUNCH(c, K_LINEARIZE, k9_linearize, dim3(cdiv(d.n_items, kWavesPerBlock)), dim3(kBlock), 0, d, c->w, huber_a);
    if (d.n_cams > 0) LAUNCH(c, K_CAM_SEGSUM, k_cam_segsum<18>, dim3(d.n_cams), dim3(kBlock), 0, c->w.scat, d.cam_ptr_g, c->w.camlin, (const PcgStatus*)nullptr);
    ReduceJobs j{};
    const double* ins[3] = {d.part, d.part + d.n_items, d.part + 2 * (size_t)d.n_items};
    double* outs[3] = {d.scal + S_COST, d.scal + S_XNORM2_PTS, d.scal + S_GRADMAX_PTS};
    for (int q = 0; q < 3; ++q) { j.in[q] = ins[q]; j.n[q] = d.n_items; j.out[q] = outs[q]; j.op[q] = q == 2 ? 1 : 0; }
    LAUNCH(c, K_SMALL, k_reduce_multi, dim3(3), dim3(kPcgThreads), 0, j);
    return 0;
}

int gradient_max_enqueue(xrsfm_ba_context* c, const Dev& d) {
    if (c->gradmax_done) { c->gradmax_done = false; return 0; }
    if (c->wide) { LAUNCH(c, K_SMALL, k9_gradmax_cams, dim3(1), dim3(kPcgThreads), 0, d, c->w, d.scal + S_GRADMAX_CAMS); return 0; }
    const double* rank_max = c->multi() ? d.camlin + (size_t)d.n_cams * 12 + 4 : nullptr;
    LAUNCH(c, K_SMALL, k_gradmax_cams, dim3(1), dim3(kPcgThreads), 0, d, d.scal + S_GRADMAX_CAMS, rank_max, c->n_ranks, d.scal + S_GRADMAX_PTS);
    return 0;
}
int gradient_max(xrsfm_ba_context* c, double* out) {
    int e = gradient_max_enqueue(c, c->d);
    if (e) return e;
    e = fetch_scalars(c);
    if (e) return e;
    *out = std::fmax(c->h_scal[S_GRADMAX_PTS], c->h_scal[S_GRADMAX_CAMS]);
    return 0;
}

int prepare_step(xrsfm_ba_context* c, double radius, bool with_blocks = false) {
    Dev& d = c->d;
    const double dmin = kLmDiagMin, dmax = kLmDiagMax;
    c->step_radius = radius;
    c->step_prep = with_blocks && c->prep_fused;
    if (c->step_prep) return 0;
    if (!with_blocks && !d.Jp) return XRSFM_BA_EINTERNAL;
    {
        const int nbp = cdiv(d.n_pts, kBlock), nbc = cdiv((long long)d.n_cams * 6, kBlock);
        if (nbp + nbc > 0) LAUNCH(c, K_SMALL, k_point_prep, dim3(nbp + nbc), dim3(kBlock), 0, d, radius, dmin, dmax, nbp);
    }
    if (with_blocks) return 0;
    if (d.n_slots > 0) LAUNCH(c, K_SCHUR_PREP, k_schur_prep, dim3(cdiv(d.n_slots, kBlock)), dim3(kBlock), 0, d);
    if (d.n_cams > 0) LAUNCH(c, K_CAM_SEGSUM, k_cam_segsum<28>, dim3(d.n_cams), dim3(kBlock), 0, d.scat, d.cam_ptr, d.camS, (const PcgStatus*)nullptr);
    int e = allreduce(c, d.camS, (size_t)d.n_cams * 28, kNcclSum);
    if (e) return e;
    if (d.n_cams > 0) LAUNCH(c, K_SMALL, k_cam_factor, dim3(cdiv(d.n_cams, 64)), dim3(64), 0, d);
    return 0;
}

int schur_product(xrsfm_ba_context* c, const double* p_dev, double* out_dev, int tag) {
    Dev& d = c->d;
    if (d.n_items > 0) { Timed t_(c, K_SCHUR_MATVEC, tag); hipLaunchKernelGGL(k_schur_matvec, dim3(cdiv(d.n_items, kWavesPerBlock)), dim3(kBlock), 0, c->stream, d, p_dev); }
    if (d.n_cams > 0) { Timed t_(c, K_CAM_SEGSUM, tag); hipLaunchKernelGGL(k_cam_segsum<6>, dim3(d.n_cams), dim3(kBlock), 0, c->stream, d.scat, d.cam_ptr, out_dev, (const PcgStatus*)d.st); }
    return allreduce(c, out_dev, (size_t)d.n_cams * 6, kNcclSum);
}

int pcg_solve(xrsfm_ba_context* c, const xrsfm_ba_options& opt, xrsfm_ba_summary* sum) {
    Dev& d = c->d;
    d.pcgW = (c->pcg_coarse && d.n_cams > 0) ? c->pcg_w : nullptr;
    if (d.pcgW && d.n_cams > 0) {
        const size_t n6 = 6 * (size_t)d.n_cams;
        d.pcgSW = c->pcg_w + kGauge * n6; d.pcgE = c->pcg_w + 2 * kGauge * n6;
        LAUNCH(c, K_PCG_VEC, k_pcg_gauge, dim3(cdiv(d.n_cams, kBlock)), dim3(kBlock), 0, d);
        HIPCHK(hipMemsetAsync(d.st, 0, sizeof(PcgStatus), c->stream));
        for (int g = 0; g < kGauge; ++g) {
            int e = schur_product(c, d.pcgW + g * n6, d.pcgSW + g * n6, -1);
            if (e) return e;
        }
// ... 309 lines not shown
                hipLaunchKernelGGL(k_gram_compact_scan, dim3(1), dim3(64), 0, c->stream, block_off, nb);
                hipLaunchKernelGGL(k_gram_compact, dim3(nb), dim3(256), 0, c->stream, cells, n_cells, h.ent_src, (const int*)block_off);
                HIPCHK(hipGetLastError());
            }
        }
    }
    h.dev.n = P.n; h.dev.n_pad = P.n_pad; h.dev.T = P.T; h.dev.cam_off = d_cam_off; h.dev.tile_rows = d_tile_rows;
    h.dev.cw = P.cam_width; h.dev.cpt = P.cams_per_tile;
    const bool packed = chol_packed_storage(P);
    h.rest_apart = chol_rest_apart(P);
    chol_plan_facts(P, h.facts);
    h.dev.tmap = packed ? d_tmap : nullptr;
    h.dev.ld = packed ? (size_t)kNB : (size_t)P.n_pad;
    h.dev.tstride = (size_t)kNB * kNB + kNB;
    h.S_doubles = packed ? ((size_t)P.n_tiles_nz + 1) * h.dev.tstride : (size_t)P.n_pad * P.n_pad;
    if (h.S_doubles * sizeof(double) > kCholMaxBytes) return XRSFM_BA_ETOOBIG;
    h.tile_map_host = P.tile_map;
    TRYC(dev_alloc(c, &h.dev.S, h.S_doubles));
    TRYC(dev_alloc(c, &h.dev.Linv, (size_t)P.T * kNB * kNB));
    TRYC(dev_alloc(c, &h.dev.y, (size_t)P.n_pad)); TRYC(dev_alloc(c, &h.dev.rhs, (size_t)P.n_pad)); TRYC(dev_alloc(c, &h.dev.x, (size_t)P.n_pad));
    {
        const BwdChoice bw = chol_bwd_choice(P);
        h.bwd_all = bw.all; h.bwd_chunk = bw.chunk; h.bwd_push = bw.push;
        { const char* te = std::getenv("XRSFM_BA_DEBUG_BWD_TIMEOUT"); h.bw_debug_timeout = te && te[0] == '1'; }
        if (h.bwd_chunk) {
            std::vector<int4> chunks;
            h.bc_off.assign(P.n_levels + 1, 0);
            int max_lv = 1;
            for (int lv = 0; lv < P.n_levels; ++lv) {
                for (int e2 = P.lv_k_off[lv]; e2 < P.lv_k_off[lv + 1]; ++e2) {
                    const int q0 = P.lv_bptr[e2], q1 = P.lv_bptr[e2 + 1];
                    const int nch = std::max(1, (q1 - q0 + kBwdChunk - 1) / kBwdChunk);
                    for (int j = 0; j < nch; ++j) chunks.push_back(make_int4(e2, q0 + j * kBwdChunk, std::min(q1, q0 + (j + 1) * kBwdChunk), j | (nch << 16)));
                }
                h.bc_off[lv + 1] = (int)chunks.size();
                max_lv = std::max(max_lv, h.bc_off[lv + 1] - h.bc_off[lv]);
            }
            TRYC(dev_upload(c, &h.bc_chunks, chunks));
            TRYC(dev_alloc(c, &h.bc_part, (size_t)max_lv * kNB)); TRYC(dev_alloc(c, &h.bc_ctr, (size_t)P.T));
            HIPCHK(hipMemsetAsync(h.bc_ctr, 0, sizeof(unsigned) * (size_t)P.T, c->stream));
        }
        if (h.bwd_all) {
            std::vector<int> order;
            std::vector<unsigned char> fin(P.T, 0);
            for (int lv = P.n_levels - 2; lv >= 0; --lv)
                for (int e2 = P.lv_k_off[lv]; e2 < P.lv_k_off[lv + 1]; ++e2) order.push_back(e2);
            for (int e2 = P.lv_k_off[P.n_levels - 1]; e2 < P.lv_k_off[P.n_levels]; ++e2) fin[P.lv_k[e2]] = 1;
            h.bw_n = (int)order.size(); h.bw_launches = 0;
            TRYC(dev_upload(c, &h.bw_order, order)); TRYC(dev_upload(c, &h.bw_final, fin));
            TRYC(dev_alloc(c, &h.bw_gx, (size_t)P.T * 2 * kNB)); TRYC(dev_alloc(c, &h.bw_ctr, (size_t)2));
            HIPCHK(hipMemsetAsync(h.bw_gx, 0, sizeof(unsigned long long) * (size_t)P.T * 2 * kNB, c->stream));
            HIPCHK(hipMemsetAsync(h.bw_ctr, 0, sizeof(unsigned) * 2, c->stream));
        }
    }
#undef TRYC
    HIPCHK(hipMemsetAsync(h.dev.S, 0, sizeof(double) * h.S_doubles, c->stream));
    const int shm = 2 * kNB * kLdT * (int)sizeof(double);
    set_kernel_attributes(c->device);
    if ((h.n_pairs_other > 0 || h.la_depth > 0) && !h.aux) {
        if (hipStreamCreateWithFlags(&h.aux, hipStreamNonBlocking) != hipSuccess) h.aux = nullptr;
        if (h.aux && (hipEventCreateWithFlags(&h.ev_fork, hipEventDisableTiming) != hipSuccess ||
                      hipEventCreateWithFlags(&h.ev_join, hipEventDisableTiming) != hipSuccess)) {
            if (h.ev_fork) (void)hipEventDestroy(h.ev_fork);
            (void)hipStreamDestroy(h.aux); h.aux = nullptr; h.ev_fork = h.ev_join = nullptr;
        }
    }
    if (h.la_depth > 0) {
        bool ok = h.aux != nullptr;
        h.la_ev_factor.assign(h.n_levels, nullptr); h.la_ev_early.assign(h.n_levels, nullptr);
        for (int lv = 0; lv < h.n_levels && ok; ++lv)
            ok = hipEventCreateWithFlags(&h.la_ev_factor[lv], hipEventDisableTiming) == hipSuccess &&
                 hipEventCreateWithFlags(&h.la_ev_early[lv], hipEventDisableTiming) == hipSuccess;
        if (!ok) {
            for (hipEvent_t e2 : h.la_ev_factor) if (e2) (void)hipEventDestroy(e2);
            for (hipEvent_t e2 : h.la_ev_early) if (e2) (void)hipEventDestroy(e2);
            h.la_ev_factor.clear(); h.la_ev_early.clear();
        }
    }
    timer.mark("allocations + attributes");
    h.ready = true;
    return 0;
}

int chol_assemble(xrsfm_ba_context* c, bool materialize = false) {
    Dev& d = c->d;
    CholHost& h = c->chol;
    const int n_obs_pairs = h.n_pairs - c->pk.n_gt_cells;
    {
        Timed t_(c, K_SCHUR_PAIRS);
        const bool fork = h.n_pairs_other > 0 && h.aux;
        const double radius = c->step_radius;
        auto launch_other = [&](hipStream_t st) {
            const int* items = h.pairs_items + h.n_pairs_small + h.n_pairs_big;
            double* pv = h.pair_from_v ? h.pair_v : nullptr;
            if (c->step_prep) hipLaunchKernelGGL((k_schur_pairs<false, true, 0>), dim3(h.n_pairs_other), dim3(kWave), h.pairs_shm, st, d, items, h.slot_pair_ptr, h.pair_dst, n_obs_pairs, h.scat2, radius, pv);
            else hipLaunchKernelGGL((k_schur_pairs<false, false, 0>), dim3(h.n_pairs_other), dim3(kWave), h.pairs_shm, st, d, items, h.slot_pair_ptr, h.pair_dst, n_obs_pairs, h.scat2, radius, pv);
        };
        auto launch_gram = [&](auto ni, int n, size_t shm, const int* items, hipStream_t st) {
            constexpr int NI = decltype(ni)::value;
            const int G = NI == 0 ? h.sgroup : 1;
            const size_t wbytes = (shm + 15) & ~(size_t)15;
            const dim3 grid(cdiv(n, G)), block(kWave * G);
            const size_t shm_wg = G > 1 ? wbytes * G : shm;
            const int wld = G > 1 ? (int)(wbytes / sizeof(double)) : 0;
            const int* sg = G > 1 ? (const int*)h.sgrp : nullptr;
            if (c->step_prep) hipLaunchKernelGGL((k_schur_pairs<true, true, NI>), grid, block, shm_wg, st, d, items, h.slot_pair_ptr, h.pair_dst, n_obs_pairs, h.scat2, radius, (double*)nullptr, h.gram4, sg, n, wld);
            else hipLaunchKernelGGL((k_schur_pairs<true, false, NI>), grid, block, shm_wg, st, d, items, h.slot_pair_ptr, h.pair_dst, n_obs_pairs, h.scat2, radius, (double*)nullptr, h.gram4, sg, n, wld);
        };
        int n_merged = 0; size_t shm_merged = 0;
        for (int b = 0; b < 6; ++b) { n_merged += h.gram_n[b]; if (h.gram_n[b] > 0) shm_merged = std::max(shm_merged, h.gram_shm[b]); }
        const bool merge = h.gram_merge && n_merged > 0;
        constexpr bool gram_fork = true;
        int big = -1;
        for (int b = 0; b < 8; ++b) if (h.gram_n[b] > 0 && (big < 0 || h.gram_n[b] > h.gram_n[big])) big = b;
        if (merge) big = -2;
        auto launch_buckets = [&](bool main_side) {
            const int* items = h.pairs_items;
            if (merge && main_side) launch_gram(std::integral_constant<int, 0>{}, n_merged, shm_merged, items, c->stream);
            for (int b = 0; b < 8; ++b) {
                const int n = h.gram_n[b];
                const bool on_main = !(fork && gram_fork) || b == big;
                if (n > 0 && on_main == main_side && !(merge && b < 6)) {
                    hipStream_t st = on_main ? c->stream : h.aux;
                    switch (b >> 1) {
                        case 0: launch_gram(std::integral_constant<int, 1>{}, n, h.gram_shm[b], items, st); break;
                        case 1: launch_gram(std::integral_constant<int, 2>{}, n, h.gram_shm[b], items, st); break;
                        case 2: launch_gram(std::integral_constant<int, 3>{}, n, h.gram_shm[b], items, st); break;
                        default: launch_gram(std::integral_constant<int, 4>{}, n, h.gram_shm[b], items, st); break;
                    }
                }
                items += n;
            }
        };
        if (fork) {
            HIPCHK(hipEventRecord(h.ev_fork, c->stream));
            launch_buckets(true);
            HIPCHK(hipStreamWaitEvent(h.aux, h.ev_fork, 0));
            launch_other(h.aux);
            launch_buckets(false);
            HIPCHK(hipEventRecord(h.ev_join, h.aux));
            HIPCHK(hipStreamWaitEvent(c->stream, h.ev_join, 0));
        } else {
            if (h.n_pairs_other > 0) launch_other(c->stream);
            launch_buckets(true);
        }
    }
    if (d.n_cams + h.n_blocks > 0) {
        if (h.pair_from_v) LAUNCH(c, K_BLOCK_SEGSUM, k_chol_segsum_v, dim3(d.n_cams + (h.n_blocks + 3) / 4), dim3(kBlock), 0, d.scat, d.cam_ptr_s, d.camS, d.n_cams, h.scat2, h.blk_ptr, h.Sblk,
                                  h.n_blocks, (const int2*)h.ent_src, (const double*)h.pair_v);
        else LAUNCH(c, K_BLOCK_SEGSUM, k_chol_segsum, dim3(d.n_cams + h.n_blocks), dim3(kBlock), 0, d.scat, d.cam_ptr_s, d.camS, d.n_cams, h.scat2, h.blk_ptr, h.Sblk);
    }
    int e = allreduce(c, d.camS, (size_t)d.n_cams * 28 + (size_t)h.n_blocks * 36, kNcclSum);
    if (e) return e;
    h.S_filled = materialize;
    if (h.S_filled && h.n_tiles_nz > 0)
        LAUNCH(c, K_DENSE_FILL, k_tile_fill, dim3(h.n_tiles_nz), dim3(256), 0, h.dev, d, h.tiles_nz, h.tf_ptr, h.tf_ent, h.Sblk, h.blk_rc,
               c->step_prep ? c->step_radius : 0.0);
    return 0;
}

static void panel_backward(xrsfm_ba_context* c) {
    CholHost& h = c->chol;
    const int T = h.T;
    int k = T - 1;
    for (int p = 0; k >= 1; k -= 2, ++p) {
            const int n = h.bw2_off[p + 1] - h.bw2_off[p];
            LAUNCH(c, K_TRISOLVE, k_bwd2, dim3(1 + n), dim3(256), 0, h.dev, k, h.bw2_link[p], (const int*)(h.bw2_ent + 2 * (size_t)h.bw2_off[p]));
        }
    for (; k >= 0; --k) {
        const int ncol = h.cols_off[k + 1] - h.cols_off[k];
        LAUNCH(c, K_TRISOLVE, k_bwd, dim3(1 + ncol), dim3(256), 0, h.dev, k, h.cols_flat + h.cols_off[k]);
    }
}

int chol_factor_solve(xrsfm_ba_context* c) {
    Dev& d = c->d;
    CholHost& h = c->chol;
    const int T = h.T;
    double* px_out = c->wide ? c->w.px : d.px;
    const size_t shm = 2 * (size_t)kNB * kLdT * sizeof(double);
    if (h.lookahead) {
        auto chunks = [&](int lv) { return lv < h.n_levels ? h.sp_chunk_off[lv + 1] - h.sp_chunk_off[lv] : 0; };
        auto targets = [&](int lv) { return lv < h.n_levels ? h.sp_rt_off[lv + 1] - h.sp_rt_off[lv] : 0; };
        auto lates = [&](int lv) { return lv < h.n_levels ? h.md_off[lv + 1] - h.md_off[lv] : 0; };
        double* const Wbuf[2] = {h.sp_work, h.sp_work + (size_t)std::max(1, h.sp_max_chunks) * kPartStride};
        double* const Qbuf[2] = {h.md_work, h.md_work + (size_t)std::max(1, h.md_max) * kPartStride};
        for (int s2 = 0; s2 < h.n_levels; ++s2) {
            const int nf = h.fz_off[s2 + 1] - h.fz_off[s2];
            SlotArgs a{};
            const int lr = s2 + 1, lp = s2 + 2;
            a.n_reduce = targets(lr);
            if (a.n_reduce > 0) { a.sp_rt = h.sp_rt + 2 * (size_t)h.sp_rt_off[lr]; a.sp_rp = h.sp_rp + 2 * (size_t)h.sp_rt_off[lr]; a.Wr = Wbuf[lr & 1]; }
            a.n_part = chunks(lp);
            if (a.n_part > 0) { a.sp_tgt = h.sp_tgt + 2 * (size_t)h.sp_chunk_off[lp]; a.sp_q = h.sp_q + 2 * (size_t)h.sp_chunk_off[lp]; a.Wp = Wbuf[lp & 1]; }
            a.n_late = lates(lr);
            if (a.n_late > 0) { a.md_tgt = h.md_tgt + 2 * (size_t)h.md_off[lr]; a.md_q = h.md_q + 2 * (size_t)h.md_off[lr]; a.Wq = Qbuf[lr & 1]; }
            if (s2 == 0 && !h.S_filled) {
                LvFill lf{};
                lf.d = d; lf.f = FillLists{h.tiles_nz, h.tf_ptr, h.tf_ent, h.Sblk, h.blk_rc, c->step_prep ? c->step_radius : 0.0};
                lf.fz_q = h.fz_q; lf.rest = h.fill_rest; lf.n_factor = nf;
                if (nf + h.n_fill_rest > 0)
                    LAUNCH(c, K_POTRF, k_lv_factor<true>, dim3(nf + h.n_fill_rest), dim3(256), 0, h.dev, h.fz_tile, h.fz_dptr, h.fz_dj,
                           (const int*)h.tile_cam, (double*)nullptr, lf);
                if (a.n_reduce + a.n_part + a.n_late > 0) return XRSFM_BA_EINTERNAL;
                continue;
            }
            a.fz_tile = h.fz_tile + 2 * (size_t)h.fz_off[s2]; a.fz_dptr = h.fz_dptr + h.fz_off[s2]; a.n_factor = nf;
            a.fz_late = h.fz_late + 2 * (size_t)h.fz_off[s2]; a.Ql = Qbuf[s2 & 1];
            const int nwg = a.n_factor + a.n_reduce + a.n_late + a.n_part;
            if (nwg > 0) LAUNCH(c, K_POTRF, k_panel_slot, dim3(nwg), dim3(256), 0, h.dev, a, (const int*)h.fz_dj, (const int*)h.lv_cj, (const int*)h.md_cj, (const int*)h.tile_cam);
        }
        panel_backward(c);
        if (d.n_cams > 0) LAUNCH(c, K_SMALL, k_sol_gather, dim3(cdiv((long long)d.n_cams * h.dev.cw, 256)), dim3(256), 0, h.dev, px_out, d.n_cams);
        return 0;
    }
    if (h.use_levels || h.panel_ll) {
        for (int lv = 0; lv < h.n_levels; ++lv) {
            const int nt = h.lv_tgt_off[lv + 1] - h.lv_tgt_off[lv];
            const int nch = h.sp_chunk_off[lv + 1] - h.sp_chunk_off[lv], nmc = h.mp_off[lv + 1] - h.mp_off[lv] - 1;
            const int nrt = h.sp_rt_off[lv + 1] - h.sp_rt_off[lv];
            const bool la_on = h.la_depth > 0 && !h.la_ev_factor.empty();
            const int n_early = la_on ? h.sp_e_cnt[lv] : 0;
            double* const Wlv = h.sp_work + (h.la_depth > 0 ? (size_t)(lv % (h.la_depth + 1)) * (size_t)std::max(1, h.sp_max_chunks) * kPartStride : 0);
            if (nmc > 0)
                LAUNCH(c, K_UPDATE, k_panel2_part, dim3(nmc), dim3(256), 0, h.dev, h.mp_chunk, h.mp_wg + h.mp_off[lv], h.sp_work);
            else if (nch - n_early > 0)
                LAUNCH(c, K_UPDATE, k_ll_update_part, dim3(nch - n_early), dim3(256), 0, h.dev, h.sp_tgt + 2 * (size_t)(h.sp_chunk_off[lv] + n_early),
                       h.sp_q + 2 * (size_t)(h.sp_chunk_off[lv] + n_early), h.lv_cj, Wlv, (const int*)(h.sp_slot + h.sp_chunk_off[lv] + n_early));
            if (n_early > 0) HIPCHK(hipStreamWaitEvent(c->stream, h.la_ev_early[lv], 0));
            if (nrt > 0)
                LAUNCH(c, K_UPDATE, k_ll_update_reduce, dim3(nrt, 16), dim3(256), 0, h.dev, h.sp_rt + 2 * (size_t)h.sp_rt_off[lv],
                       h.sp_rp + 2 * (size_t)h.sp_rt_off[lv], Wlv);
            const int nf = h.fz_off[lv + 1] - h.fz_off[lv];
            const bool with_bwd = ((!h.panel_ll && !h.bwd_push && !h.bwd_chunk) || T == 1) && lv == h.n_levels - 1;
            LvFill lf{};
            if (lv == 0 && !h.S_filled) {
                lf.d = d; lf.f = FillLists{h.tiles_nz, h.tf_ptr, h.tf_ent, h.Sblk, h.blk_rc, c->step_prep ? c->step_radius : 0.0};
                lf.fz_q = h.fz_q; lf.rest = h.fill_rest; lf.n_factor = nf;
                const bool rest_apart = h.rest_apart;
                if (rest_apart)
                    LAUNCH(c, K_DENSE_FILL, k_tile_fill, dim3(h.n_fill_rest), dim3(256), 0, h.dev, d, h.tiles_nz, h.tf_ptr, h.tf_ent, h.Sblk, h.blk_rc,
                           c->step_prep ? c->step_radius : 0.0, (const int*)h.fill_rest);
                const int n_rest = rest_apart ? 0 : h.n_fill_rest;
                if (nf + n_rest > 0)
                    LAUNCH(c, K_POTRF, k_lv_factor<true>, dim3(nf + n_rest), dim3(256), 0, h.dev, h.fz_tile, h.fz_dptr, h.fz_dj,
                           (const int*)h.tile_cam, with_bwd ? px_out : (double*)nullptr, lf);
            } else if (nf > 0)
                LAUNCH(c, K_POTRF, k_lv_factor<false>, dim3(nf), dim3(256), 0, h.dev, h.fz_tile + 2 * (size_t)h.fz_off[lv], h.fz_dptr + h.fz_off[lv], h.fz_dj,
                       (const int*)h.tile_cam, with_bwd ? px_out : (double*)nullptr, lf);
            if (la_on) {
                const int le = lv + 1 + h.la_depth;
                const int ne = le < h.n_levels ? h.sp_e_cnt[le] : 0;
                if (ne > 0) {
                    HIPCHK(hipEventRecord(h.la_ev_factor[lv], c->stream));
                    HIPCHK(hipStreamWaitEvent(h.aux, h.la_ev_factor[lv], 0));
                    double* const Wle = h.sp_work + (size_t)(le % (h.la_depth + 1)) * (size_t)std::max(1, h.sp_max_chunks) * kPartStride;
                    {
                        Timed t_(c, K_UPDATE, -1, h.aux);
                        hipLaunchKernelGGL(k_ll_update_part, dim3(ne), dim3(256), 0, h.aux, h.dev, h.sp_tgt + 2 * (size_t)h.sp_chunk_off[le],
                                           h.sp_q + 2 * (size_t)h.sp_chunk_off[le], h.lv_cj, Wle, (const int*)(h.sp_slot + h.sp_chunk_off[le]));
                    }
                    HIPCHK(hipEventRecord(h.la_ev_early[le], h.aux));
                }
            }
        }
        if (h.panel_ll || h.bwd_push) {
            if (T == 1) return 0;
            panel_backward(c);
            if (d.n_cams > 0) LAUNCH(c, K_SMALL, k_sol_gather, dim3(cdiv((long long)d.n_cams * h.dev.cw, 256)), dim3(256), 0, h.dev, px_out, d.n_cams);
            return 0;
        }
        if (h.bwd_chunk) {
            for (int lv = h.n_levels - 1; lv >= 0; --lv) {
                const int n = h.bc_off[lv + 1] - h.bc_off[lv];
                if (n > 0) LAUNCH(c, K_TRISOLVE, k_lv_bwd_chunk, dim3(n), dim3(256), 0, h.dev, (const int*)h.lv_k, (const int*)h.lv_bi, (const int*)h.tile_cam, px_out,
                                  (const int4*)(h.bc_chunks + h.bc_off[lv]), h.bc_part, h.bc_ctr);
            }
            return 0;
        }
        if (h.bwd_all && h.bw_n > 0) {
            const unsigned base = h.bw_launches * (unsigned)h.bw_n;
            const unsigned epoch = ++h.bw_launches;
            LAUNCH(c, K_TRISOLVE, k_lv_bwd_all, dim3(h.bw_n), dim3(256), 0, h.dev, (const int*)h.lv_k, (const int*)h.lv_bptr, (const int*)h.lv_bi,
                   (const int*)h.tile_cam, px_out, (const int*)h.bw_order, (const unsigned char*)h.bw_final, h.bw_gx, h.bw_ctr, base, epoch, h.bw_ctr + 1,
                   d.scal + S_BWD_ERR, h.bw_debug_timeout ? 64u : kBwdSpinMax, h.bw_debug_timeout ? epoch + 1u : epoch);
            return 0;
        }
        for (int lv = h.n_levels - 2; lv >= 0; --lv) {
            const int nk = h.lv_k_off[lv + 1] - h.lv_k_off[lv];
            LAUNCH(c, K_TRISOLVE, k_lv_bwd, dim3(nk), dim3(256), 0, h.dev, h.lv_k + h.lv_k_off[lv], h.lv_bptr + h.lv_k_off[lv], h.lv_bi, h.tile_cam, px_out);
        }
        return 0;
    }
    return XRSFM_BA_EINTERNAL;
}

Dev candidate_view(const xrsfm_ba_context* c) {
    Dev v = c->d;
    std::swap(v.cam, v.cam_cand); std::swap(v.P, v.P_cand);
    v.rt = c->alt.rt; v.Jp = c->alt.Jp; v.camrec = c->alt.camrec; v.Hpp = c->alt.Hpp; v.gp = c->alt.gp; v.camlin = c->alt.camlin;
    v.part = c->d.part + 4 * (size_t)c->d.n_items;
    return v;
}
void accept_candidate(xrsfm_ba_context* c) {
    Dev& d = c->d;
    std::swap(d.cam, d.cam_cand); std::swap(d.P, d.P_cand);
    std::swap(d.rt, c->alt.rt); std::swap(d.Jp, c->alt.Jp); std::swap(d.camrec, c->alt.camrec);
    std::swap(d.Hpp, c->alt.Hpp); std::swap(d.gp, c->alt.gp); std::swap(d.camlin, c->alt.camlin);
}

int finish_step(xrsfm_ba_context* c, double huber_a, bool speculate) {
    Dev& d = c->d;
    const bool cams_done = c->fused;
    if (c->wide) {
        const int nbi = cdiv(d.n_items, kWavesPerBlock), nbc = cdiv(d.n_cams, kBlock);
        if (nbi + nbc > 0) LAUNCH(c, K_BACKSUB, k9_backsub, dim3(nbi + nbc), dim3(kBlock), 0, d, c->w, nbi, c->step_radius);
    } else {
        const int nbi = cdiv(d.n_items, kWavesPerBlock), nbc = cams_done ? cdiv(d.n_cams, kBlock) : 0;
        CamLin* cr = (cams_done && speculate) ? c->alt.camrec : (CamLin*)nullptr;
        if (nbi + nbc > 0) {
            if (c->step_prep) LAUNCH(c, K_BACKSUB, k_backsub<true>, dim3(nbi + nbc), dim3(kBlock), 0, d, nbi, cr, c->step_radius);
            else LAUNCH(c, K_BACKSUB, k_backsub<false>, dim3(nbi + nbc), dim3(kBlock), 0, d, nbi, cr, c->step_radius);
        }
        if (d.n_cams > 0 && !cams_done) LAUNCH(c, K_SMALL, k_cam_update, dim3(cdiv(d.n_cams, kBlock)), dim3(kBlock), 0, d);
    }
    if (speculate) {
        const Dev cand = candidate_view(c);
        int e = linearize(c, huber_a, cand, true, LIN_FINAL | (cams_done ? LIN_SKIP_CAMLIN : 0));
        if (e) return e;
        if ((e = gradient_max_enqueue(c, cand))) return e;
        return fetch_scalars(c);
    }
    if (d.n_items > 0) LAUNCH(c, K_COST, k_cost, dim3(cdiv(d.n_items, kWavesPerBlock)), dim3(kBlock), 0, d, huber_a);
    {
        ReduceJobs j{};
        const double* ins[5] = {d.part, d.part + 2 * (size_t)d.n_items, d.part + 3 * (size_t)d.n_items, d.campart, d.campart + d.n_cams};
        const int ns[5] = {d.n_items, d.n_items, d.n_items, d.n_cams, d.n_cams};
        double* outs[5] = {d.scal + S_COST_CAND, d.scal + S_MODEL, d.scal + S_STEP2_PTS, d.scal + S_STEP2_CAMS, d.scal + S_XNORM2_CAMS};
        for (int q = 0; q < 5; ++q) { j.in[q] = ins[q]; j.n[q] = ns[q]; j.out[q] = outs[q]; j.op[q] = 0; }
        LAUNCH(c, K_SMALL, k_reduce_multi, dim3(5), dim3(kPcgThreads), 0, j);
    }
    int e = allreduce(c, d.scal + S_MODEL, 3, kNcclSum);
    if (e) return e;
    return fetch_scalars(c);
}

int bwd_all_status(xrsfm_ba_context* c) {
    CholHost& h = c->chol;
    if (!h.bwd_all || h.bw_launches == 0 || !h.bw_ctr) return 0;
    unsigned ev = 0;
    if (hipMemcpy(&ev, h.bw_ctr + 1, sizeof(unsigned), hipMemcpyDeviceToHost) != hipSuccess) return XRSFM_BA_ENODEV;
    if (ev) {
        fprintf(stderr, "[xrsfm_ba] backward substitution: a hand-off between workgroups timed out (k_lv_bwd_all); rerun with XRSFM_BA_BWD_ALL=0\n");
        (void)hipMemset(h.bw_ctr + 1, 0, sizeof(unsigned));
        return XRSFM_BA_EINTERNAL;
    }
    return 0;
}

void print_progress(const xrsfm_ba_options& o, int it, double cost, double change, double gmax, double step, double rho, double radius) {
    if (!o.verbose) return;
    if (it == 0) printf("iter      cost      cost_change  |gradient|   |step|    tr_ratio  tr_radius\n");
    printf("%4d  %.6e  %9.2e  %9.2e  %9.2e  %9.2e  %9.2e\n", it, cost, change, gmax, step, rho, radius);
}

int init_scaling_and_linearize(xrsfm_ba_context* c, double huber_a, bool use_scaling) {
    Dev& d = c->d;
    const int cw = c->wide ? kW : 6;
    int e;
    LAUNCH(c, K_SMALL, k_fill, dim3(cdiv((long long)d.n_cams * cw, kBlock) + 1), dim3(kBlock), 0, c->wide ? c->w.scale_c : d.scale_c, 1.0, (size_t)d.n_cams * cw);
    LAUNCH(c, K_SMALL, k_fill, dim3(cdiv((long long)d.n_pts * 3, kBlock) + 1), dim3(kBlock), 0, d.scale_p, 1.0, (size_t)d.n_pts * 3);
    c->gradmax_done = false; c->published = false;
    auto lin = [&](int flags) { return c->wide ? linearize_wide(c, huber_a) : linearize(c, huber_a, d, false, flags); };
    if ((e = lin(use_scaling ? 0 : LIN_FINAL))) return e;
    if (use_scaling) {
        const long long n = std::max((long long)d.n_cams * cw, (long long)d.n_pts * 3);
        if (c->wide) LAUNCH(c, K_SMALL, k9_scale_from_norms, dim3(cdiv(n, kBlock) + 1), dim3(kBlock), 0, d, c->w);
        else LAUNCH(c, K_SMALL, k_scale_from_norms, dim3(cdiv(n, kBlock) + 1), dim3(kBlock), 0, d);
        if ((e = lin(LIN_FINAL))) return e;
    }
    c->linearized = true;
    return 0;
}

struct DevScratch {
    std::vector<void*> p;
    ~DevScratch() { for (void* q : p) (void)hipFree(q); }
    template <typename T>
    int get(T** out, size_t n) {
        void* q = nullptr;
        if (hipMalloc(&q, std::max<size_t>(1, n) * sizeof(T)) != hipSuccess) return XRSFM_BA_ENOMEM;
        p.push_back(q); *out = static_cast<T*>(q);
        return 0;
    }
    template <typename T>
    int put(T** out, const std::vector<T>& v) {
        if (int e = get(out, v.size())) return e;
        if (!v.empty() && hipMemcpy(*out, v.data(), v.size() * sizeof(T), hipMemcpyHostToDevice) != hipSuccess) return XRSFM_BA_ENODEV;
        return 0;
    }
};

static int cov_solution_status(xrsfm_ba_context* c, std::vector<double>& x) {
    x.resize((size_t)c->d.n_cams * 6);
    HIPCHK(hipMemcpyAsync(x.data(), c->d.px, x.size() * sizeof(double), hipMemcpyDeviceToHost, c->stream));
    HIPCHK(hipStreamSynchronize(c->stream));
    if (int e = bwd_all_status(c)) return e;
    for (double v : x) if (!std::isfinite(v)) return XRSFM_BA_ESINGULAR;
    return 0;
}

struct CovLists {
    std::vector<int4> ent; std::vector<int2> lj; std::vector<int> sel_row, sel_cam;
// ... 572 lines not shown
    }
    if (d.n_cams + h.n_blocks > 0) LAUNCH(c, K_BLOCK_SEGSUM, k9_chol_segsum, dim3(d.n_cams + h.n_blocks), dim3(kBlock), 0, c->w.scat, d.cam_ptr_g, c->w.camS, d.n_cams, h.scat2, h.blk_ptr, h.Sblk);
    if (h.n_tiles_nz > 0) LAUNCH(c, K_DENSE_FILL, k9_tile_fill, dim3(h.n_tiles_nz), dim3(256), 0, h.dev, d, c->w, h.tiles_nz, h.tf_ptr, h.tf_ent, h.Sblk, h.blk_rc, radius);
    h.S_filled = true;
    return 0;
}

static int ba_run_impl(xrsfm_ba_context* c, const xrsfm_ba_options* optp, xrsfm_ba_summary* sum) {
    if (!c || !optp || !sum) return XRSFM_BA_EINVAL;
    if (c->poisoned) return XRSFM_BA_ESTATE;
    const xrsfm_ba_options opt = *optp;
    HIPCHK(hipSetDevice(c->device));
    if (const char* se = std::getenv("XRSFM_BA_DEBUG_STALL_S"))
        c->debug_stall_ticks = (unsigned long long)(std::fmin(std::fmax(std::atof(se), 0.0), 10.0) * 1e8);
    memset(sum, 0, sizeof(*sum));
    Dev& d = c->d;
    hipStream_t st = c->stream;
    int solver = opt.linear_solver;
    int e;
    if (c->wide) {
        if (solver == XRSFM_BA_SOLVER_PCG || c->multi()) {
            fprintf(stderr, "[xrsfm_ba] variable intrinsics (9-wide camera blocks): only the exact solver on one rank is implemented\n");
            return XRSFM_BA_EINVAL;
        }
        solver = XRSFM_BA_SOLVER_CHOLESKY;
    }
    if (solver == XRSFM_BA_SOLVER_AUTO) {
        try { e = chol_setup(c); } catch (const std::bad_alloc&) { e = XRSFM_BA_ENOMEM; }
        if (e == XRSFM_BA_ETOOBIG || e == XRSFM_BA_ENOMEM || e == kErrDuplicateObs) solver = XRSFM_BA_SOLVER_PCG;
        else if (e) return e;
        else solver = XRSFM_BA_SOLVER_CHOLESKY;
    }
    if (solver != XRSFM_BA_SOLVER_PCG && solver != XRSFM_BA_SOLVER_CHOLESKY) return XRSFM_BA_EINVAL;
    if (solver == XRSFM_BA_SOLVER_CHOLESKY && (e = chol_setup(c))) {
        if (e == kErrDuplicateObs) {
            fprintf(stderr, "[xrsfm_ba] a track is observed twice by one camera: the explicit reduced camera matrix is not available, use AUTO or PCG\n");
            return XRSFM_BA_EINVAL;
        }
        return e;
    }
    if ((e = use_stored_j(c, !jfree_for_run(c, solver)))) return e;
    sum->linear_solver_used = solver;
    c->profiling = opt.profile != 0;
    for (int i = 0; i < K_COUNT; ++i) { c->prof_ms[i] = 0.0; c->prof_n[i] = 0; }
    c->recs.clear(); c->ev_used = 0;
    const auto t_begin = std::chrono::steady_clock::now();
    sum->num_residuals = 2 * c->pk.n_obs;
    {
        int n_var_i = 0;
        if (c->wide && d.n_cams) {
            std::vector<unsigned char> cc(d.n_cams);
            std::vector<double> act(d.n_cams);
            HIPCHK(hipMemcpy(cc.data(), d.cam_const, d.n_cams, hipMemcpyDeviceToHost)); HIPCHK(hipMemcpy(act.data(), d.cam_act, sizeof(double) * d.n_cams, hipMemcpyDeviceToHost));
            for (int i = 0; i < d.n_cams; ++i) n_var_i += (act[i] > 0.0 && (cc[i] & kCamIntrVariable)) ? 1 : 0;
        }
        sum->num_effective_params = 3 * (c->pk.n_var_q + c->pk.n_var_t + c->pk.n_var_p + n_var_i);
    }
    auto finish = [&](int term, int reason, double cost) {
        sum->termination = term; sum->termination_reason = reason; sum->final_cost = cost;
        (void)hipStreamSynchronize(st);
        sum->total_time_s = std::chrono::duration<double>(std::chrono::steady_clock::now() - t_begin).count();
        if (int be = bwd_all_status(c)) return be;
        if (c->profiling) {
            profile_collect(c);
            int best = 0;
            for (int i = 1; i < K_COUNT - 1; ++i) if (c->prof_ms[i] > c->prof_ms[best]) best = i;
            sum->dom_kernel_id = best; sum->dom_kernel_ms = c->prof_ms[best]; sum->dom_kernel_launches = c->prof_n[best];
        }
        c->profiling = false;
        return XRSFM_BA_OK;
    };
    if ((e = init_scaling_and_linearize(c, opt.huber_a, true))) return e;
    double gmax = 0.0;
    if ((e = gradient_max(c, &gmax))) return e;
    double cost = 0.5 * c->h_scal[S_COST];
    double xnorm2_pts = c->h_scal[S_XNORM2_PTS];
    sum->initial_cost = cost;
    xtr::TrustRegion tr{opt.initial_radius};
    print_progress(opt, 0, cost, 0.0, gmax, 0.0, 0.0, tr.radius);
    if (gmax <= opt.gradient_tolerance) return finish(XRSFM_BA_CONVERGENCE, 1, cost);
    int it = 0;
    bool speculate = !c->wide;
    int accepted_run = 0;
    while (true) {
        if (it >= opt.max_iterations) return finish(XRSFM_BA_NO_CONVERGENCE, 5, cost);
        ++it;
        sum->lm_steps_attempted++;
        if (c->wide) {
            if ((e = assemble_wide(c, tr.radius))) return e;
            if ((e = chol_factor_solve(c))) return e;
        } else {
            if ((e = prepare_step(c, tr.radius, solver == XRSFM_BA_SOLVER_CHOLESKY))) return e;
            if (solver == XRSFM_BA_SOLVER_PCG) {
                if ((e = pcg_solve(c, opt, sum))) return e;
            } else {
                if ((e = chol_assemble(c))) return e;
                if ((e = chol_factor_solve(c))) return e;
            }
        }
        if ((e = finish_step(c, opt.huber_a, speculate))) return e;
        const double* s = c->h_scal;
        const double model_change = s[S_MODEL];
        const double xnorm = std::sqrt(xnorm2_pts + s[S_XNORM2_CAMS]);
        if (!(model_change > 0.0) || !std::isfinite(model_change)) {
            sum->n_unsuccessful++;
            print_progress(opt, it, cost, 0.0, gmax, 0.0, 0.0, tr.radius);
            if (const int r = tr.invalid_step()) return finish(XRSFM_BA_FAILURE, r, cost);
            if (!d.Jp && (e = use_stored_j(c, true, true))) return e;
            continue;
        }
        tr.invalid = 0;
        const double cost_cand = 0.5 * (speculate ? s[S_COST] : s[S_COST_CAND]);
        const double step_norm = std::sqrt(s[S_STEP2_PTS] + s[S_STEP2_CAMS]);
        const double cost_change = cost - cost_cand;
        if (const int r = xtr::TrustRegion::tolerance_exit(step_norm, xnorm, opt.parameter_tolerance, cost_change, cost, opt.function_tolerance))
            return finish(XRSFM_BA_CONVERGENCE, r, cost);
        const double rel = cost_change / model_change;
        if (xtr::TrustRegion::successful(rel)) {
            if (speculate) {
                accept_candidate(c);
                cost = cost_cand;
                xnorm2_pts = s[S_XNORM2_PTS];
                gmax = std::fmax(s[S_GRADMAX_PTS], s[S_GRADMAX_CAMS]);
            } else {
                std::swap(d.cam, d.cam_cand);
                std::swap(d.P, d.P_cand);
                if ((e = c->wide ? linearize_wide(c, opt.huber_a) : linearize(c, opt.huber_a, d, false, LIN_FINAL))) return e;
                if ((e = gradient_max(c, &gmax))) return e;
                cost = 0.5 * c->h_scal[S_COST];
                xnorm2_pts = c->h_scal[S_XNORM2_PTS];
            }
            ++accepted_run;
            speculate = !c->wide && (sum->n_unsuccessful == 0 || accepted_run >= 2);
            tr.grow(rel);
            sum->n_successful++;
            print_progress(opt, it, cost, cost_change, gmax, step_norm, rel, tr.radius);
            if (gmax <= opt.gradient_tolerance) return finish(XRSFM_BA_CONVERGENCE, 1, cost);
        } else {
            speculate = false; accepted_run = 0;
            const int r = tr.shrink();
            if (!d.Jp && (e = use_stored_j(c, true, true))) return e;
            sum->n_unsuccessful++;
            print_progress(opt, it, cost, cost_change, gmax, step_norm, rel, tr.radius);
            if (r) return finish(XRSFM_BA_CONVERGENCE, r, cost);
        }
    }
}

int xrsfm_ba_profile_entry(xrsfm_ba_context* c, int index, const char** name, double* total_ms, int* launches) {
    if (!c || index < 0 || index >= K_COUNT) return XRSFM_BA_EINVAL;
    if (name) *name = kKidName[index];
    if (total_ms) *total_ms = c->prof_ms[index];
    if (launches) *launches = c->prof_n[index];
    return 0;
}

int xrsfm_ba_solve(const xrsfm_ba_options* opt, xrsfm_ba_problem* problem, xrsfm_ba_summary* summary) {
    if (!opt || !problem || !summary) return XRSFM_BA_EINVAL;
    static const bool trace = std::getenv("XRSFM_BA_TRACE_CALLS") != nullptr;
    using clk = std::chrono::steady_clock;
    const auto t0 = clk::now();
    xrsfm_ba_context* c = nullptr;
    int e = xrsfm_ba_create(problem, 0, &c);
    if (e) return e;
    const auto t1 = clk::now();
    e = xrsfm_ba_run(c, opt, summary);
    const auto t2 = clk::now();
    if (!e) e = xrsfm_ba_download(c, problem->cam_q, problem->cam_t, problem->points);
    if (!e && problem->intr_params) e = xrsfm_ba_download_intrinsics(c, problem->intr_params);
    const auto t3 = clk::now();
    xrsfm_ba_destroy(c);
    if (trace) {
        auto ms = [](clk::time_point a, clk::time_point b) { return std::chrono::duration<double, std::milli>(b - a).count(); };
        std::fprintf(stderr, "[xrsfm_ba_solve] cams %d points %d obs %d | create %.3f run %.3f download %.3f destroy %.3f ms | LM %d+%d solver %d rc %d\n",
                     problem->n_cams, problem->n_points, problem->n_obs, ms(t0, t1), ms(t1, t2), ms(t2, t3), ms(t3, clk::now()),
                     summary->n_successful, summary->n_unsuccessful, summary->linear_solver_used, e);
    }
    return e;
}

void xrsfm_pg_default_options(xrsfm_pg_options* o) {
    if (!o) return;
    o->max_iterations = 100; o->function_tolerance = 1e-6; o->parameter_tolerance = 1e-8; o->gradient_tolerance = 1e-10;
    o->initial_radius = 1e16; o->verbose = 0; o->bounds_active_set = 0;
}

static int pg_solve_impl(const xrsfm_pg_options* opt, xrsfm_pg_problem* p, xrsfm_pg_summary* summary) {
    if (!p || !summary) return XRSFM_BA_EINVAL;
    if (p->n_frames < 0 || p->n_scales < p->n_frames || p->n_edges < 0 || p->n_scale_costs < 0) return XRSFM_BA_EINVAL;
    if (p->n_frames > 0 && (!p->rot_q || !p->pos)) return XRSFM_BA_EINVAL;
    if (p->n_scales > 0 && !p->scale) return XRSFM_BA_EINVAL;
    if (p->n_edges > 0 && (!p->edge_a || !p->edge_b || !p->edge_sa || !p->edge_sb || !p->edge_q_mea || !p->edge_p_mea)) return XRSFM_BA_EINVAL;
    if (p->n_scale_costs > 0 && (!p->sc_a || !p->sc_b || !p->sc_s12)) return XRSFM_BA_EINVAL;
    for (int e = 0; e < p->n_edges; ++e) {
        if (p->edge_a[e] < 0 || p->edge_a[e] >= p->n_frames || p->edge_b[e] < 0 || p->edge_b[e] >= p->n_frames) return XRSFM_BA_EINVAL;
        if (p->edge_sa[e] < 0 || p->edge_sa[e] >= p->n_scales || p->edge_sb[e] < 0 || p->edge_sb[e] >= p->n_scales) return XRSFM_BA_EINVAL;
    }
    for (int e = 0; e < p->n_scale_costs; ++e)
        if (p->sc_a[e] < 0 || p->sc_a[e] >= p->n_scales || p->sc_b[e] < 0 || p->sc_b[e] >= p->n_scales) return XRSFM_BA_EINVAL;
    xrsfm_pg_options o;
    if (opt) o = *opt; else xrsfm_pg_default_options(&o);
    xpg::Solver solver(*p);
    return solver.run(o, summary);
}

void xrsfm_tag_default_options(xrsfm_pg_options* o) {
    if (!o) return;
    o->max_iterations = 500;
    o->function_tolerance = 1e-6; o->parameter_tolerance = 1e-8; o->gradient_tolerance = 1e-10;
    o->initial_radius = 1e4; o->verbose = 0; o->bounds_active_set = 0;
}

static int tag_refine_impl(const xrsfm_pg_options* opt, xrsfm_tag_problem* p, int32_t stages, xrsfm_pg_summary* summaries) {
    if (!p || !summaries || stages < 1 || stages > 2) return XRSFM_BA_EINVAL;
    if (p->n_frames < 0 || p->n_tags < 0 || p->n_tag_obs < 0 || p->n_points < 0 || p->n_obs < 0) return XRSFM_BA_EINVAL;
    if (p->n_frames > 0 && (!p->frame_q || !p->frame_t)) return XRSFM_BA_EINVAL;
    if (p->n_tags > 0 && (!p->tag_corners || !p->tag_q || !p->tag_t)) return XRSFM_BA_EINVAL;
    if (p->n_tag_obs > 0 && (!p->tag_obs_tag || !p->tag_obs_frame || !p->tag_obs_xy)) return XRSFM_BA_EINVAL;
    if (p->n_points > 0 && !p->points) return XRSFM_BA_EINVAL;
    if (p->n_obs > 0 && (!p->obs_frame || !p->obs_pt || !p->obs_xy)) return XRSFM_BA_EINVAL;
    if (!(p->tag_length > 0.0) || !std::isfinite(p->scale)) return XRSFM_BA_EINVAL;
    for (int i = 0; i < p->n_tag_obs; ++i)
        if (p->tag_obs_tag[i] < 0 || p->tag_obs_tag[i] >= p->n_tags || p->tag_obs_frame[i] < 0 || p->tag_obs_frame[i] >= p->n_frames) return XRSFM_BA_EINVAL;
    for (int i = 0; i < p->n_obs; ++i)
        if (p->obs_pt[i] < 0 || p->obs_pt[i] >= p->n_points || p->obs_frame[i] < 0 || p->obs_frame[i] >= p->n_frames) return XRSFM_BA_EINVAL;
    xrsfm_pg_options o;
    if (opt) o = *opt; else xrsfm_tag_default_options(&o);
    return xtag::refine(o, *p, stages, summaries);
}
// ... 755 lines not shown
```

Measured before the change: 1.127 billion.

## Decide LM step acceptance on device and queue next Schur assembly ahead

Moves the Levenberg-Marquardt accept/reject and trust-region update into the final linearization tail kernel. It writes a go word keyed by the sequence number so the next iteration's Schur-pair and segment-sum kernels can be enqueued speculatively before the host reads the scalars. Those kernels exit early when the device decides not to continue, and the radius is read from device memory. This hides the host round trip between iterations, at the cost of bit-exact replication of the host trust-region arithmetic on device, with a fallback to the host when rounding could differ.

New measurement: 1.124 billion. Within noise of the previous version (-0.3%).

```diff
diff --git a/include/xrsfm_ba.h b/include/xrsfm_ba.h
--- a/include/xrsfm_ba.h
+++ b/include/xrsfm_ba.h
@@ -227,6 +227,9 @@
 
 int xrsfm_ba_debug_stored_j(xrsfm_ba_context *ctx, int32_t *stored);
 
+int xrsfm_ba_debug_lm_stats(xrsfm_ba_context *ctx, int32_t *decided_on_device, int32_t *queued_ahead, int32_t *cancelled);
+int xrsfm_ba_debug_lm_decide(int32_t n, const double *scal, const double *state, double *out_device, double *out_host);
+
 #ifdef __cplusplus
 }
 #endif
diff --git a/xrsfm_amd/capi.py b/xrsfm_amd/capi.py
--- a/xrsfm_amd/capi.py
+++ b/xrsfm_amd/capi.py
@@ -84,7 +84,7 @@
     "xrsfm_ba_debug_cholesky_solve", "xrsfm_ba_debug_set_block_pattern", "xrsfm_ba_debug_pack", "xrsfm_ba_debug_chol_plan", "xrsfm_ba_refine_pose", "xrsfm_ba_refine_pose_options", "xrsfm_ba_debug_comm_hook", "xrsfm_pg_default_options", "xrsfm_pg_solve", "xrsfm_ba_debug_pack_gram", "xrsfm_ba_debug_gram_schedule",
     "xrsfm_tag_default_options", "xrsfm_tag_refine", "xrsfm_ba_refine_poses", "xrsfm_ba_quiesce", "xrsfm_ba_debug_backsub", "xrsfm_ba_device_memory", "xrsfm_ba_download_intrinsics", "xrsfm_ba_debug_wide",
     "xrsfm_ba_debug_device_pack_check", "xrsfm_ba_warmup", "xrsfm_ba_debug_stored_j", "xrsfm_ba_debug_sgroup",
-    "xrsfm_ba_debug_reduced_system", "xrsfm_ba_covariance",
+    "xrsfm_ba_debug_reduced_system", "xrsfm_ba_covariance", "xrsfm_ba_debug_lm_stats", "xrsfm_ba_debug_lm_decide",
 ]
 
 CHOL_FACTS = ("T", "levels", "ordering", "schedule", "macro_levels", "split_levels", "la_depth", "fill_rest", "rest_apart", "packed",
@@ -180,6 +180,11 @@
     lib.xrsfm_ba_profile_entry.restype = C.c_int
     lib.xrsfm_ba_covariance.argtypes = [vp, C.c_double, C.c_int32, _c_int32_p, _c_double_p]
     lib.xrsfm_ba_covariance.restype = C.c_int
+    if hasattr(lib, "xrsfm_ba_debug_lm_stats"):
+        lib.xrsfm_ba_debug_lm_stats.argtypes = [vp] + [C.POINTER(C.c_int32)] * 3
+        lib.xrsfm_ba_debug_lm_stats.restype = C.c_int
+        lib.xrsfm_ba_debug_lm_decide.argtypes = [C.c_int32] + [_c_double_p] * 4
+        lib.xrsfm_ba_debug_lm_decide.restype = C.c_int
     _lib = lib
     return lib
 
@@ -206,6 +211,16 @@
     lib.xrsfm_ba_quiesce.restype = C.c_int
     check(lib.xrsfm_ba_quiesce(C.byref(n)), "xrsfm_ba_quiesce")
     return int(n.value)
+
+
+def debug_lm_decide(scal, state):
+    scal = np.ascontiguousarray(scal, np.float64).reshape(-1, 16)
+    state = np.ascontiguousarray(state, np.float64).reshape(-1, 10)
+    n = scal.shape[0]
+    assert state.shape[0] == n
+    dev = np.zeros((n, 8)); host = np.zeros((n, 8))
+    check(load().xrsfm_ba_debug_lm_decide(n, _dp(scal), _dp(state), _dp(dev), _dp(host)), "debug_lm_decide")
+    return dev, host
 
 
 def default_options(**kw) -> COptions:
@@ -349,6 +364,11 @@
         v = C.c_int32(0)
         check(self.lib.xrsfm_ba_debug_stored_j(self._h, C.byref(v)), "debug_stored_j")
         return bool(v.value)
+
+    def debug_lm_stats(self) -> dict:
+        v = [C.c_int32(0) for _ in range(3)]
+        check(self.lib.xrsfm_ba_debug_lm_stats(self._h, *(C.byref(x) for x in v)), "debug_lm_stats")
+        return dict(zip(("decided", "queued", "cancelled"), (int(x.value) for x in v)))
 
     def debug_cholesky_solve(self, radius: float, want_S: bool = False):
         n = 6 * self.problem.n_cams
diff --git a/xrsfm_amd/csrc/ba_chol.h b/xrsfm_amd/csrc/ba_chol.h
--- a/xrsfm_amd/csrc/ba_chol.h
+++ b/xrsfm_amd/csrc/ba_chol.h
@@ -310,9 +310,12 @@
 __global__ __launch_bounds__((GRAM && NIK == 0) ? kWave * kSGroupMax : kWave) __attribute__((amdgpu_waves_per_eu((GRAM && NIK < 4) ? 4 : (GRAM ? 3 : 2), (GRAM && NIK < 4) ? 4 : 3)))
 void k_schur_pairs(Dev d, const int* __restrict__ item_list, const int* __restrict__ slot_pair_ptr, const int* __restrict__ pair_dst,
                    int n_obs_pairs, double* __restrict__ scat2, double radius, double* __restrict__ pair_v = nullptr, int gram4 = 1,
-                   const int* __restrict__ sgrp = nullptr, int n_list = 0, int wld = 0) {
+                   const int* __restrict__ sgrp = nullptr, int n_list = 0, int wld = 0,
+                   const double* __restrict__ radius_p = nullptr, const unsigned long long* __restrict__ go = nullptr, unsigned long long expect = 0) {
     extern __shared__ __attribute__((aligned(16))) double smem_all[];
     constexpr bool MERGED = GRAM && NIK == 0;
+    if (go && *go != expect) return;
+    if (radius_p) radius = *radius_p;
     const int lane = MERGED ? (int)__builtin_amdgcn_mbcnt_hi(~0u, __builtin_amdgcn_mbcnt_lo(~0u, 0u)) : (int)threadIdx.x;
     const int wave = MERGED ? __builtin_amdgcn_readfirstlane((int)(threadIdx.x >> 6)) : 0;
     const int pos = MERGED ? (int)blockIdx.x * (int)(blockDim.x >> 6) + wave : (int)blockIdx.x;
diff --git a/xrsfm_amd/csrc/ba_kernels.h b/xrsfm_amd/csrc/ba_kernels.h
--- a/xrsfm_amd/csrc/ba_kernels.h
+++ b/xrsfm_amd/csrc/ba_kernels.h
@@ -1,5 +1,6 @@
 #pragma once
 #include "ba_math.h"
+#include "ba_trust_region.h"
 
 namespace xba {
 
@@ -23,8 +24,75 @@
     S_COST = 0, S_XNORM2_PTS, S_MODEL, S_STEP2_PTS, S_COST_CAND, S_STEP2_CAMS, S_XNORM2_CAMS,
     S_GRADMAX_PTS, S_GRADMAX_CAMS,
     S_BWD_ERR,
+    S_LM_GO,
+    S_LM_RADIUS,
+    S_LM_DECREASE,
+    S_LM_CODE,
     S_COUNT = 16
 };
+
+struct LmState {
+    double radius, decrease;
+    double cost, xnorm2_pts;
+    double function_tolerance, parameter_tolerance, gradient_tolerance;
+    int invalid;
+    int it, max_iterations;
+    int pad;
+};
+enum LmBranch { LM_HOST = 0, LM_INVALID = 1, LM_TOLERANCE = 2, LM_ACCEPT = 3, LM_REJECT = 4 };
+
+__device__ __host__ inline int lm_decide(const double* sc, LmState& st, bool* go) {
+#ifdef __clang__
+#pragma clang fp contract(off)
+#endif
+    *go = false;
+    if (sc[S_BWD_ERR] != 0.0) return 0;
+    xtr::TrustRegion tr{st.radius, st.decrease, st.invalid};
+    const double model_change = sc[S_MODEL];
+    const double xnorm = std::sqrt(st.xnorm2_pts + sc[S_XNORM2_CAMS]);
+    int branch, reason = 0;
+    if (!(model_change > 0.0) || !std::isfinite(model_change)) {
+        branch = LM_INVALID;
+        reason = tr.invalid_step();
+    } else {
+        tr.invalid = 0;
+        const double cost_cand = 0.5 * sc[S_COST];
+        const double step_norm = std::sqrt(sc[S_STEP2_PTS] + sc[S_STEP2_CAMS]);
+        const double cost_change = st.cost - cost_cand;
+        if ((reason = xtr::TrustRegion::tolerance_exit(step_norm, xnorm, st.parameter_tolerance, cost_change, st.cost, st.function_tolerance)))
+            branch = LM_TOLERANCE;
+        else {
+            const double rel = cost_change / model_change;
+            if (xtr::TrustRegion::successful(rel)) {
+                if (!tr.grow_as_host(rel)) return 0;
+                branch = LM_ACCEPT;
+                st.cost = cost_cand;
+                st.xnorm2_pts = sc[S_XNORM2_PTS];
+                if (std::fmax(sc[S_GRADMAX_PTS], sc[S_GRADMAX_CAMS]) <= st.gradient_tolerance) reason = 1;
+                else if (st.it >= st.max_iterations) reason = 5;
+                *go = reason == 0;
+            } else {
+                branch = LM_REJECT;
+                reason = tr.shrink();
+            }
+        }
+    }
+    st.radius = tr.radius; st.decrease = tr.decrease; st.invalid = tr.invalid;
+    ++st.it;
+    return branch | reason << 4 | tr.invalid << 8;
+}
+
+__global__ void k_lm_set(LmState* out, LmState v) { *out = v; }
+
+__global__ void k_lm_decide_debug(const double* __restrict__ sc, LmState* st, double* __restrict__ out, int n) {
+    const int i = blockIdx.x * blockDim.x + threadIdx.x;
+    if (i >= n) return;
+    LmState s = st[i];
+    bool go = false;
+    const int code = lm_decide(sc + (size_t)S_COUNT * i, s, &go);
+    st[i] = s;
+    out[4 * i] = go ? 1.0 : 0.0; out[4 * i + 1] = s.radius; out[4 * i + 2] = s.decrease; out[4 * i + 3] = (double)code;
+}
 
 struct __attribute__((aligned(16))) CamLin {
     double M[9];
@@ -581,7 +649,9 @@
 
 __global__ __launch_bounds__(kBlock) void k_chol_segsum(const double* __restrict__ scat, const int* __restrict__ cam_ptr,
                                                         double* __restrict__ camS, int n_cams, const double* __restrict__ scat2,
-                                                        const int* __restrict__ blk_ptr, double* __restrict__ Sblk) {
+                                                        const int* __restrict__ blk_ptr, double* __restrict__ Sblk,
+                                                        const unsigned long long* __restrict__ go = nullptr, unsigned long long expect = 0) {
+    if (go && *go != expect) return;
     if ((int)blockIdx.x < n_cams) segsum_body<28>(scat, cam_ptr, camS, blockIdx.x);
     else segsum_body<36>(scat2, blk_ptr, Sblk, blockIdx.x - n_cams);
 }
@@ -624,7 +694,9 @@
 __global__ __launch_bounds__(kBlock) void k_chol_segsum_v(const double* __restrict__ scat, const int* __restrict__ cam_ptr,
                                                           double* __restrict__ camS, int n_cams, const double* __restrict__ scat2,
                                                           const int* __restrict__ blk_ptr, double* __restrict__ Sblk, int n_blocks,
-                                                          const int2* __restrict__ ent_src, const double* __restrict__ pair_v) {
+                                                          const int2* __restrict__ ent_src, const double* __restrict__ pair_v,
+                                                          const unsigned long long* __restrict__ go = nullptr, unsigned long long expect = 0) {
+    if (go && *go != expect) return;
     if ((int)blockIdx.x < n_cams) { segsum_body<28>(scat, cam_ptr, camS, blockIdx.x); return; }
     constexpr int K = 36, NW = kBlock / kWave;
     __shared__ double ops[NW][kPairVAhead][K];
@@ -1538,6 +1610,7 @@
     unsigned* ticket;
     int gradmax;
     double* host; unsigned long long seq;
+    LmState* lm;
 };
 
 constexpr int kTailJobs = 8;
@@ -1613,6 +1686,18 @@
     __syncthreads();
     if (t < 9) __hip_atomic_store(a.ticket + 32 * t, 0u, __ATOMIC_RELAXED, __HIP_MEMORY_SCOPE_AGENT);
     if (a.host) {
+        if (a.lm) {
+            if (t == 0) {
+                LmState st = *a.lm;
+                bool go = false;
+                const int code = lm_decide(sc, st, &go);
+                if (code) *a.lm = st;
+                sc[S_LM_GO] = __longlong_as_double(go ? (long long)a.seq : 0ll);
+                sc[S_LM_RADIUS] = st.radius; sc[S_LM_DECREASE] = st.decrease; sc[S_LM_CODE] = (double)code;
+            }
+            __syncthreads();
+            if (t >= S_LM_GO && t <= S_LM_CODE) d.scal[t] = sc[t];
+        }
         if (t < S_COUNT) a.host[t] = sc[t];
         __threadfence_system();
         __syncthreads();
diff --git a/xrsfm_amd/csrc/ba_trust_region.h b/xrsfm_amd/csrc/ba_trust_region.h
--- a/xrsfm_amd/csrc/ba_trust_region.h
+++ b/xrsfm_amd/csrc/ba_trust_region.h
@@ -6,6 +6,11 @@
 #define XTR_HD __host__ __device__
 #else
 #define XTR_HD
+#endif
+#ifdef __clang__
+#define XTR_NO_CONTRACT _Pragma("clang fp contract(off)")
+#else
+#define XTR_NO_CONTRACT
 #endif
 
 namespace xtr {
@@ -21,21 +26,46 @@
     int invalid = 0;
 
     XTR_HD int invalid_step() {
+        XTR_NO_CONTRACT
         if (++invalid >= kMaxInvalidSteps) return 6;
         radius /= decrease; decrease *= 2.0;
         return 0;
     }
     XTR_HD static int tolerance_exit(double step_norm, double xnorm, double ptol, double cost_change, double cost, double ftol) {
+        XTR_NO_CONTRACT
         if (step_norm <= ptol * (xnorm + ptol)) return 2;
         if (std::fabs(cost_change) <= ftol * cost) return 3;
         return 0;
     }
     XTR_HD static bool successful(double rho) { return rho > kMinRelDecrease; }
     XTR_HD void grow(double rho) {
+        XTR_NO_CONTRACT
         radius = std::fmin(kMaxRadius, radius / std::fmax(1.0 / 3.0, 1.0 - std::pow(2.0 * rho - 1.0, 3)));
         decrease = 2.0;
     }
+    XTR_HD bool grow_as_host(double rho) {
+        XTR_NO_CONTRACT
+#ifdef __HIP_DEVICE_COMPILE__
+        const double t = 2.0 * rho - 1.0, at = std::fabs(t);
+        if (!(t == 0.0 || (at > 1e-100 && at < 1e100))) return false;
+        const double p = t * t, pe = __builtin_fma(t, t, -p);
+        const double h = p * t, he = __builtin_fma(p, t, -h);
+        const double l = he + pe * t;
+        const double r = h + l, rem = (h - r) + l;
+        const double den = std::fmax(1.0 / 3.0, 1.0 - r);
+        const double below = std::nextafter(r, -HUGE_VAL), above = std::nextafter(r, HUGE_VAL);
+        const bool same = std::fmax(1.0 / 3.0, 1.0 - below) == den && std::fmax(1.0 / 3.0, 1.0 - above) == den;
+        if (!same && !(std::fabs(rem) < 0.45 * std::fabs((rem > 0.0 ? above : below) - r))) return false;
+        radius = std::fmin(kMaxRadius, radius / den);
+        decrease = 2.0;
+        return true;
+#else
+        grow(rho);
+        return true;
+#endif
+    }
     XTR_HD int shrink() {
+        XTR_NO_CONTRACT
         radius /= decrease; decrease *= 2.0;
         return radius < kMinRadius ? 4 : 0;
     }
diff --git a/xrsfm_amd/csrc/xrsfm_ba.hip b/xrsfm_amd/csrc/xrsfm_ba.hip
--- a/xrsfm_amd/csrc/xrsfm_ba.hip
+++ b/xrsfm_amd/csrc/xrsfm_ba.hip
@@ -172,6 +172,8 @@
     bool step_valid = false;
     bool gradmax_done = false, published = false;
     double* part2 = nullptr; unsigned* ticket = nullptr;
+    LmState* lm_state = nullptr; bool lm_fresh = false; LmState* lm_next = nullptr;
+    int lm_decided = 0, lm_queued = 0, lm_cancelled = 0;
     struct LinBuf { double* rt = nullptr; double* Jp = nullptr; CamLin* camrec = nullptr; double* Hpp = nullptr; double* gp = nullptr; double* camlin = nullptr; } alt;
     double* jbuf[4] = {nullptr, nullptr, nullptr, nullptr};
     std::vector<unsigned long long> pattern_keys;
@@ -535,7 +537,8 @@
             a.jobs = j; a.njobs = nj; a.part2 = c->part2; a.ticket = c->ticket;
             const bool final_here = (flags & LIN_FINAL) && !multi;
             a.gradmax = final_here ? 1 : 0;
-            if (final_here && !c->profiling && c->h_scal_dev) { a.host = c->h_scal_dev; a.seq = ++c->seq; c->published = true; }
+            if (final_here && !c->profiling && c->h_scal_dev) { a.host = c->h_scal_dev; a.seq = ++c->seq; c->published = true; a.lm = c->lm_next; }
+            c->lm_next = nullptr;
             LAUNCH(c, K_SMALL, k_lin_tail, dim3(std::min(kTailGrid, std::max(d.n_cams, 1))), dim3(kBlock), 0, d, a);
             if (final_here) c->gradmax_done = true;
         } else {
@@ -1011,10 +1014,13 @@
     return 0;
 }
 
-int chol_assemble(xrsfm_ba_context* c, bool materialize = false) {
-    Dev& d = c->d;
+int chol_assemble(xrsfm_ba_context* c, bool materialize = false, const Dev* view = nullptr, unsigned long long expect = 0) {
+    const Dev& d = view ? *view : c->d;
     CholHost& h = c->chol;
     const int n_obs_pairs = h.n_pairs - c->pk.n_gt_cells;
+    const double* radius_p = view ? d.scal + S_LM_RADIUS : nullptr;
+    const unsigned long long* go = view ? reinterpret_cast<const unsigned long long*>(d.scal + S_LM_GO) : nullptr;
+    if (view && (materialize || c->multi() || !c->step_prep)) return XRSFM_BA_EINTERNAL;
     {
         Timed t_(c, K_SCHUR_PAIRS);
         const bool fork = h.n_pairs_other > 0 && h.aux;
@@ -1022,8 +1028,8 @@
         auto launch_other = [&](hipStream_t st) {
             const int* items = h.pairs_items + h.n_pairs_small + h.n_pairs_big;
             double* pv = h.pair_from_v ? h.pair_v : nullptr;
-            if (c->step_prep) hipLaunchKernelGGL((k_schur_pairs<false, true, 0>), dim3(h.n_pairs_other), dim3(kWave), h.pairs_shm, st, d, items, h.slot_pair_ptr, h.pair_dst, n_obs_pairs, h.scat2, radius, pv);
-            else hipLaunchKernelGGL((k_schur_pairs<false, false, 0>), dim3(h.n_pairs_other), dim3(kWave), h.pairs_shm, st, d, items, h.slot_pair_ptr, h.pair_dst, n_obs_pairs, h.scat2, radius, pv);
+            if (c->step_prep) hipLaunchKernelGGL((k_schur_pairs<false, true, 0>), dim3(h.n_pairs_other), dim3(kWave), h.pairs_shm, st, d, items, h.slot_pair_ptr, h.pair_dst, n_obs_pairs, h.scat2, radius, pv, 1, (const int*)nullptr, 0, 0, radius_p, go, expect);
+            else hipLaunchKernelGGL((k_schur_pairs<false, false, 0>), dim3(h.n_pairs_other), dim3(kWave), h.pairs_shm, st, d, items, h.slot_pair_ptr, h.pair_dst, n_obs_pairs, h.scat2, radius, pv, 1, (const int*)nullptr, 0, 0, radius_p, go, expect);
         };
         auto launch_gram = [&](auto ni, int n, size_t shm, const int* items, hipStream_t st) {
             constexpr int NI = decltype(ni)::value;
@@ -1033,8 +1039,8 @@
             const size_t shm_wg = G > 1 ? wbytes * G : shm;
             const int wld = G > 1 ? (int)(wbytes / sizeof(double)) : 0;
             const int* sg = G > 1 ? (const int*)h.sgrp : nullptr;
-            if (c->step_prep) hipLaunchKernelGGL((k_schur_pairs<true, true, NI>), grid, block, shm_wg, st, d, items, h.slot_pair_ptr, h.pair_dst, n_obs_pairs, h.scat2, radius, (double*)nullptr, h.gram4, sg, n, wld);
-            else hipLaunchKernelGGL((k_schur_pairs<true, false, NI>), grid, block, shm_wg, st, d, items, h.slot_pair_ptr, h.pair_dst, n_obs_pairs, h.scat2, radius, (double*)nullptr, h.gram4, sg, n, wld);
+            if (c->step_prep) hipLaunchKernelGGL((k_schur_pairs<true, true, NI>), grid, block, shm_wg, st, d, items, h.slot_pair_ptr, h.pair_dst, n_obs_pairs, h.scat2, radius, (double*)nullptr, h.gram4, sg, n, wld, radius_p, go, expect);
+            else hipLaunchKernelGGL((k_schur_pairs<true, false, NI>), grid, block, shm_wg, st, d, items, h.slot_pair_ptr, h.pair_dst, n_obs_pairs, h.scat2, radius, (double*)nullptr, h.gram4, sg, n, wld, radius_p, go, expect);
         };
         int n_merged = 0; size_t shm_merged = 0;
         for (int b = 0; b < 6; ++b) { n_merged += h.gram_n[b]; if (h.gram_n[b] > 0) shm_merged = std::max(shm_merged, h.gram_shm[b]); }
@@ -1076,8 +1082,8 @@
     }
     if (d.n_cams + h.n_blocks > 0) {
         if (h.pair_from_v) LAUNCH(c, K_BLOCK_SEGSUM, k_chol_segsum_v, dim3(d.n_cams + (h.n_blocks + 3) / 4), dim3(kBlock), 0, d.scat, d.cam_ptr_s, d.camS, d.n_cams, h.scat2, h.blk_ptr, h.Sblk,
-                                  h.n_blocks, (const int2*)h.ent_src, (const double*)h.pair_v);
-        else LAUNCH(c, K_BLOCK_SEGSUM, k_chol_segsum, dim3(d.n_cams + h.n_blocks), dim3(kBlock), 0, d.scat, d.cam_ptr_s, d.camS, d.n_cams, h.scat2, h.blk_ptr, h.Sblk);
+                                  h.n_blocks, (const int2*)h.ent_src, (const double*)h.pair_v, go, expect);
+        else LAUNCH(c, K_BLOCK_SEGSUM, k_chol_segsum, dim3(d.n_cams + h.n_blocks), dim3(kBlock), 0, d.scat, d.cam_ptr_s, d.camS, d.n_cams, h.scat2, h.blk_ptr, h.Sblk, go, expect);
     }
     int e = allreduce(c, d.camS, (size_t)d.n_cams * 28 + (size_t)h.n_blocks * 36, kNcclSum);
     if (e) return e;
@@ -1238,7 +1244,7 @@
     std::swap(d.Hpp, c->alt.Hpp); std::swap(d.gp, c->alt.gp); std::swap(d.camlin, c->alt.camlin);
 }
 
-int finish_step(xrsfm_ba_context* c, double huber_a, bool speculate) {
+int finish_step(xrsfm_ba_context* c, double huber_a, bool speculate, bool queue_ahead = false) {
     Dev& d = c->d;
     const bool cams_done = c->fused;
     if (c->wide) {
@@ -1258,6 +1264,13 @@
         int e = linearize(c, huber_a, cand, true, LIN_FINAL | (cams_done ? LIN_SKIP_CAMLIN : 0));
         if (e) return e;
         if ((e = gradient_max_enqueue(c, cand))) return e;
+        if (queue_ahead) {
+            if (!c->published) return XRSFM_BA_EINTERNAL;
+            Dev next = cand;
+            next.part = d.part; next.huber_a = d.huber_a;
+            if ((e = chol_assemble(c, false, &next, c->seq))) return e;
+            c->lm_queued++;
+        }
         return fetch_scalars(c);
     }
     if (d.n_items > 0) LAUNCH(c, K_COST, k_cost, dim3(cdiv(d.n_items, kWavesPerBlock)), dim3(kBlock), 0, d, huber_a);
@@ -1996,6 +2009,12 @@
     int it = 0;
     bool speculate = !c->wide;
     int accepted_run = 0;
+    const bool dev_allowed = [] { const char* de = std::getenv("XRSFM_BA_DEVICE_DECISION"); return !(de && de[0] == '0'); }() &&
+                             !c->wide && !c->multi() && solver == XRSFM_BA_SOLVER_CHOLESKY && c->fused && !c->profiling && c->h_scal_dev;
+    c->lm_decided = c->lm_queued = c->lm_cancelled = 0;
+    c->lm_fresh = false; c->lm_next = nullptr;
+    if (dev_allowed && !c->lm_state && (e = dev_alloc(c, &c->lm_state, 1))) return e;
+    bool queued = false;
     while (true) {
         if (it >= opt.max_iterations) return finish(XRSFM_BA_NO_CONVERGENCE, 5, cost);
         ++it;
@@ -2008,29 +2027,58 @@
             if (solver == XRSFM_BA_SOLVER_PCG) {
                 if ((e = pcg_solve(c, opt, sum))) return e;
             } else {
-                if ((e = chol_assemble(c))) return e;
+                if (!queued && (e = chol_assemble(c))) return e;
                 if ((e = chol_factor_solve(c))) return e;
             }
         }
-        if ((e = finish_step(c, opt.huber_a, speculate))) return e;
+        queued = false;
+        const bool dev_decide = dev_allowed && speculate && c->step_prep && !c->debug_stall_ticks;
+        if (dev_decide) {
+            if (!c->lm_fresh) {
+                LmState ls{};
+                ls.radius = tr.radius; ls.decrease = tr.decrease; ls.invalid = tr.invalid;
+                ls.cost = cost; ls.xnorm2_pts = xnorm2_pts;
+                ls.function_tolerance = opt.function_tolerance; ls.parameter_tolerance = opt.parameter_tolerance; ls.gradient_tolerance = opt.gradient_tolerance;
+                ls.it = it; ls.max_iterations = opt.max_iterations;
+                LAUNCH(c, K_SMALL, k_lm_set, dim3(1), dim3(1), 0, c->lm_state, ls);
+            }
+            c->lm_next = c->lm_state;
+        }
+        const unsigned long long handover = c->seq + 1;
+        e = finish_step(c, opt.huber_a, speculate, dev_decide);
+        c->lm_next = nullptr;
+        if (e) return e;
         const double* s = c->h_scal;
+        int dev_code = 0;
+        if (dev_decide) {
+            unsigned long long go_word;
+            memcpy(&go_word, s + S_LM_GO, sizeof go_word);
+            dev_code = (int)s[S_LM_CODE];
+            queued = go_word == handover;
+            if (!queued) c->lm_cancelled++;
+            if (queued != ((dev_code & 15) == LM_ACCEPT && ((dev_code >> 4) & 15) == 0)) return XRSFM_BA_EINTERNAL;
+            if (dev_code) { tr.radius = s[S_LM_RADIUS]; tr.decrease = s[S_LM_DECREASE]; tr.invalid = dev_code >> 8; c->lm_decided++; }
+        }
+        c->lm_fresh = dev_code != 0;
+        const int dev_branch = dev_code & 15, dev_reason = (dev_code >> 4) & 15;
         const double model_change = s[S_MODEL];
         const double xnorm = std::sqrt(xnorm2_pts + s[S_XNORM2_CAMS]);
-        if (!(model_change > 0.0) || !std::isfinite(model_change)) {
+        if (dev_code ? dev_branch == LM_INVALID : (!(model_change > 0.0) || !std::isfinite(model_change))) {
             sum->n_unsuccessful++;
-            print_progress(opt, it, cost, 0.0, gmax, 0.0, 0.0, tr.radius);
-            if (const int r = tr.invalid_step()) return finish(XRSFM_BA_FAILURE, r, cost);
+            print_progress(opt, it, cost, 0.0, gmax, 0.0, 0.0, dev_code ? c->step_radius : tr.radius);
+            if (const int r = dev_code ? dev_reason : tr.invalid_step()) return finish(XRSFM_BA_FAILURE, r, cost);
             if (!d.Jp && (e = use_stored_j(c, true, true))) return e;
             continue;
         }
-        tr.invalid = 0;
+        if (!dev_code) tr.invalid = 0;
         const double cost_cand = 0.5 * (speculate ? s[S_COST] : s[S_COST_CAND]);
         const double step_norm = std::sqrt(s[S_STEP2_PTS] + s[S_STEP2_CAMS]);
         const double cost_change = cost - cost_cand;
-        if (const int r = xtr::TrustRegion::tolerance_exit(step_norm, xnorm, opt.parameter_tolerance, cost_change, cost, opt.function_tolerance))
+        if (const int r = dev_code ? (dev_branch == LM_TOLERANCE ? dev_reason : 0)
+                                   : xtr::TrustRegion::tolerance_exit(step_norm, xnorm, opt.parameter_tolerance, cost_change, cost, opt.function_tolerance))
             return finish(XRSFM_BA_CONVERGENCE, r, cost);
         const double rel = cost_change / model_change;
-        if (xtr::TrustRegion::successful(rel)) {
+        if (dev_code ? dev_branch == LM_ACCEPT : xtr::TrustRegion::successful(rel)) {
             if (speculate) {
                 accept_candidate(c);
                 cost = cost_cand;
@@ -2046,19 +2094,62 @@
             }
             ++accepted_run;
             speculate = !c->wide && (sum->n_unsuccessful == 0 || accepted_run >= 2);
-            tr.grow(rel);
+            if (!dev_code) tr.grow(rel);
             sum->n_successful++;
             print_progress(opt, it, cost, cost_change, gmax, step_norm, rel, tr.radius);
-            if (gmax <= opt.gradient_tolerance) return finish(XRSFM_BA_CONVERGENCE, 1, cost);
+            if (dev_code ? dev_reason == 1 : gmax <= opt.gradient_tolerance) return finish(XRSFM_BA_CONVERGENCE, 1, cost);
         } else {
             speculate = false; accepted_run = 0;
-            const int r = tr.shrink();
+            const int r = dev_code ? dev_reason : tr.shrink();
             if (!d.Jp && (e = use_stored_j(c, true, true))) return e;
             sum->n_unsuccessful++;
             print_progress(opt, it, cost, cost_change, gmax, step_norm, rel, tr.radius);
             if (r) return finish(XRSFM_BA_CONVERGENCE, r, cost);
         }
     }
+}
+
+int xrsfm_ba_debug_lm_stats(xrsfm_ba_context* c, int32_t* decided_on_device, int32_t* queued_ahead, int32_t* cancelled) {
+    if (!c) return XRSFM_BA_EINVAL;
+    if (decided_on_device) *decided_on_device = c->lm_decided;
+    if (queued_ahead) *queued_ahead = c->lm_queued;
+    if (cancelled) *cancelled = c->lm_cancelled;
+    return 0;
+}
+
+int xrsfm_ba_debug_lm_decide(int32_t n, const double* scal, const double* state, double* out_device, double* out_host) {
+    if (n < 0 || (n > 0 && (!scal || !state || !out_device || !out_host))) return XRSFM_BA_EINVAL;
+    if (n == 0) return 0;
+    std::vector<LmState> st(n);
+    for (int i = 0; i < n; ++i) {
+        const double* q = state + 10 * (size_t)i;
+        LmState& l = st[i];
+        l.radius = q[0]; l.decrease = q[1]; l.cost = q[2]; l.xnorm2_pts = q[3];
+        l.function_tolerance = q[4]; l.parameter_tolerance = q[5]; l.gradient_tolerance = q[6];
+        l.invalid = (int)q[7]; l.it = (int)q[8]; l.max_iterations = (int)q[9]; l.pad = 0;
+    }
+    auto put = [](double* o, bool go, int code, const LmState& l) {
+        o[0] = go ? 1.0 : 0.0; o[1] = l.radius; o[2] = l.decrease; o[3] = (double)code; o[4] = l.cost; o[5] = l.xnorm2_pts; o[6] = l.invalid; o[7] = l.it;
+    };
+    for (int i = 0; i < n; ++i) {
+        LmState l = st[i];
+        bool go = false;
+        const int code = lm_decide(scal + (size_t)S_COUNT * i, l, &go);
+        put(out_host + 8 * (size_t)i, go, code, l);
+    }
+    DevScratch ds;
+    double* d_sc = nullptr; LmState* d_st = nullptr; double* d_out = nullptr;
+    int e;
+    if ((e = ds.get(&d_sc, (size_t)n * S_COUNT)) || (e = ds.get(&d_st, (size_t)n)) || (e = ds.get(&d_out, (size_t)n * 4))) return e;
+    HIPCHK(hipMemcpy(d_sc, scal, sizeof(double) * (size_t)n * S_COUNT, hipMemcpyHostToDevice));
+    HIPCHK(hipMemcpy(d_st, st.data(), sizeof(LmState) * (size_t)n, hipMemcpyHostToDevice));
+    hipLaunchKernelGGL(k_lm_decide_debug, dim3(cdiv(n, 64)), dim3(64), 0, nullptr, d_sc, d_st, d_out, n);
+    HIPCHK(hipGetLastError());
+    std::vector<double> o4((size_t)n * 4);
+    HIPCHK(hipMemcpy(o4.data(), d_out, sizeof(double) * o4.size(), hipMemcpyDeviceToHost));
+    HIPCHK(hipMemcpy(st.data(), d_st, sizeof(LmState) * (size_t)n, hipMemcpyDeviceToHost));
+    for (int i = 0; i < n; ++i) put(out_device + 8 * (size_t)i, o4[4 * (size_t)i] != 0.0, (int)o4[4 * (size_t)i + 3], st[i]);
+    return 0;
 }
 
 int xrsfm_ba_profile_entry(xrsfm_ba_context* c, int index, const char** name, double* total_ms, int* launches) {
```
